# UmbertoDellaMonica/fp-mash

Hardware: AMD Instinct MI355X
Metric: bases/s sketched + Mpairs/s dist, k=21 s=1000, 1/2/4/8 MI355X; %HBM roofline (higher is better)
Workload: dtype u64; 1 GPU; n_seqs_per_gpu=10000, seq_len=2000, k=21, s=1000, pairs_per_gpu=100000000, listed_pairs_per_gpu=1000006, full=False

## Files before the change

fp-mash_amd/csrc/dist.hip:

```cpp
#include "fpm_device.hpp"
#include "fpm_kernels.hpp"

#pragma clang fp contract(off)

#include <cstdlib>

#include <float.h>

#include <algorithm>

namespace fpm {

constexpr int kTile = 16;
constexpr int kWalkBlk = 4;

template <typename H>
__device__ __forceinline__ void walk_pair(const H *__restrict__ A, uint32_t la,
                                          const H *__restrict__ B, uint32_t lb, uint32_t S,
                                          uint32_t &numer, uint32_t &denom)
{
    uint32_t i = 0, j = 0, common = 0, d = 0;
    H a = la ? A[0] : H(0), b = lb ? B[0] : H(0);
    while (d < S && i < la && j < lb) {
        const bool lt = a < b, gt = b < a;
        if (!gt) { i++; if (i < la) a = A[i]; }
        if (!lt) { j++; if (j < lb) b = B[j]; }
        common += (!lt && !gt) ? 1u : 0u;
        d++;
    }
    if (d < S) {
        uint64_t dd = (uint64_t)d + (la - i) + (lb - j);
        d = dd > S ? S : (uint32_t)dd;
    }
    numer = common;
    denom = d;
}

template <typename H, typename C>
__global__ __launch_bounds__(256) void compare_grid_kernel(
    const H *__restrict__ ref, const uint32_t *__restrict__ ref_len, uint64_t ref_stride,
    uint32_t n_ref, const H *__restrict__ qry, const uint32_t *__restrict__ qry_len,
    uint64_t qry_stride, uint32_t n_qry, uint32_t S, C *__restrict__ numer,
    C *__restrict__ denom)
{
    const uint32_t r = blockIdx.x * kTile + (threadIdx.x & (kTile - 1));
    const uint32_t q = blockIdx.y * kTile + (threadIdx.x / kTile);
    if (r >= n_ref || q >= n_qry) return;
    uint32_t c, d;
    walk_pair(ref + (uint64_t)r * ref_stride, ref_len[r], qry + (uint64_t)q * qry_stride,
              qry_len[q], S, c, d);
    const uint64_t o = (uint64_t)q * n_ref + r;
    numer[o] = (C)c;
    denom[o] = (C)d;
}

__device__ __forceinline__ uint32_t lane_sel(uint32_t x, uint32_t y, uint64_t m)
{
    uint32_t r;
    asm("v_cndmask_b32_e64 %0, %1, %2, %3" : "=v"(r) : "v"(x), "v"(y), "s"(m));
    return r;
}
__device__ __forceinline__ uint64_t lane_sel(uint64_t x, uint64_t y, uint64_t m)
{
    return ((uint64_t)lane_sel((uint32_t)(x >> 32), (uint32_t)(y >> 32), m) << 32) |
           lane_sel((uint32_t)x, (uint32_t)y, m);
}

template <typename H, int BLK, typename C>
__global__ __launch_bounds__(256) void compare_grid_lds_kernel(
    const H *__restrict__ ref, const uint32_t *__restrict__ ref_len, uint64_t ref_stride,
    uint32_t n_ref, const H *__restrict__ qry, const uint32_t *__restrict__ qry_len,
    uint64_t qry_stride, uint32_t n_qry, uint32_t S, uint32_t W, C *__restrict__ numer,
    C *__restrict__ denom)
{
    extern __shared__ __attribute__((aligned(16))) unsigned char smem[];
    H *lds = reinterpret_cast<H *>(smem);
    __shared__ uint32_t cnt[2 * kTile];
    const uint32_t Wp = (W + BLK + 3) & ~3u;
    const uint32_t r0 = blockIdx.x * kTile, q0 = blockIdx.y * kTile;
    if (threadIdx.x < 2 * kTile) {
        const uint32_t l = threadIdx.x, isq = l >= (uint32_t)kTile, row = (isq ? q0 : r0) + (l & (kTile - 1));
        uint32_t c = 0;
        if (row < (isq ? n_qry : n_ref)) c = isq ? qry_len[row] : ref_len[row];
        cnt[l] = c < W ? c : W;
    }
    __syncthreads();
    const uint32_t wave = threadIdx.x >> 6, lane = threadIdx.x & 63;
    constexpr uint32_t kV = 16 / sizeof(H);
    constexpr int kL = 2 * kTile / 4;
    const bool vec = ((ref_stride * sizeof(H)) & 15) == 0 && ((qry_stride * sizeof(H)) & 15) == 0 &&
                     (((uintptr_t)ref | (uintptr_t)qry) & 15) == 0;
    if (vec) {
// ... 107 lines not shown
        if (++x < na) ra = RA[x];
        if (++y < nb) rb = RB[y];
    }
    numer = common;
    const uint64_t dd = (uint64_t)la + lb - common;
    denom = dd > S ? S : (uint32_t)dd;
}

template <typename H, typename C>
__global__ __launch_bounds__(256) void walk_cand_kernel(
    const uint64_t *__restrict__ cand, const unsigned long long *__restrict__ n_cand,
    const H *__restrict__ ref, const uint32_t *__restrict__ ref_len, uint64_t ref_stride,
    uint32_t n_ref, const H *__restrict__ qry, const uint32_t *__restrict__ qry_len,
    uint64_t qry_stride, uint32_t S, RecRows rr, RecRows rq, C *__restrict__ numer,
    C *__restrict__ denom)
{
    const uint64_t idx = (uint64_t)blockIdx.x * blockDim.x + threadIdx.x;
    if (idx >= *n_cand) return;
    const uint64_t o = cand[idx];
    const uint32_t q = (uint32_t)(o / n_ref), r = (uint32_t)(o % n_ref);
    uint32_t c, d;
    const H *A = ref + (uint64_t)r * ref_stride, *B = qry + (uint64_t)q * qry_stride;
    if (A == B && ref_len[r] == qry_len[q]) {
        const uint32_t l = ref_len[r];
        c = l < S ? l : S;
        const uint64_t dd = 2ull * l - c;
        d = dd > S ? S : (uint32_t)dd;
    } else if (rr.val)
        walk_pair_rec(ref + (uint64_t)r * ref_stride, ref_len[r], qry + (uint64_t)q * qry_stride,
                      qry_len[q], S, (const H *)rr.val + (uint64_t)r * rr.stride,
                      rr.pos + (uint64_t)r * rr.stride, rr.len[r],
                      (const H *)rq.val + (uint64_t)q * rq.stride, rq.pos + (uint64_t)q * rq.stride,
                      rq.len[q], c, d);
    else
        walk_pair(ref + (uint64_t)r * ref_stride, ref_len[r], qry + (uint64_t)q * qry_stride,
                  qry_len[q], S, c, d);
    numer[o] = (C)c;
    denom[o] = (C)d;
}

constexpr int kRankWaves = 4;
constexpr int kRankProbeMax = 8;
constexpr uint32_t kRankLogB = 12;

template <int NP, bool HI = false>
__device__ __forceinline__ uint64_t rank_chunk(const uint64_t *Bs, const uint32_t *K32,
                                               const uint16_t *Bkt, uint32_t shift,
                                               uint32_t kshift, uint32_t top, uint32_t lb,
                                               uint32_t maxn, uint32_t kb, uint64_t a, uint32_t &j)
{
    bool over;
    uint32_t lo;
    if constexpr (HI) {
        over = false;
        lo = Bkt[min((uint32_t)(a >> 32) >> (shift - 32), kb)];
    } else {
        const uint64_t t = a >> shift;
        over = t > (uint64_t)top;
        lo = Bkt[over ? top + 1 : (uint32_t)t];
    }
    if constexpr (NP > 0) {
        const uint32_t ka = HI ? (uint32_t)(a >> 32) : (uint32_t)(a >> kshift);
        uint32_t p = lo;
#pragma unroll
        for (int q = 0; q < NP; q++) p += K32[lo + q] < ka ? 1u : 0u;
        const uint64_t v = Bs[p];
        j = p + (v < a ? 1u : 0u);
        if constexpr (HI) return __builtin_amdgcn_ballot_w64(v == a);
        return __builtin_amdgcn_ballot_w64(v == a) & ~__builtin_amdgcn_ballot_w64(over);
    } else {
        uint32_t jj = lo;
        uint64_t eqm = 0;
        for (uint32_t q = 0; q < maxn; q++) {
            const uint32_t p = min(lo + q, lb);
            const uint64_t v = Bs[p];
            jj += ((v < a) & (p < lb)) ? 1u : 0u;
            eqm |= __builtin_amdgcn_ballot_w64((v == a) & (p < lb));
        }
        j = jj;
        return eqm;
    }
}

template <int CAP, typename C>
__global__ __launch_bounds__(64 * kRankWaves) void rank_rows_kernel(
    const uint64_t *__restrict__ cand, const uint64_t *__restrict__ row_seg, uint32_t n_qry,
    uint32_t q_lo, const uint64_t *__restrict__ ref, const uint32_t *__restrict__ ref_len,
    uint64_t ref_stride, uint32_t n_ref, const uint64_t *__restrict__ qry,
    const uint32_t *__restrict__ qry_len, uint64_t qry_stride, uint32_t S, uint32_t sym,
    C *__restrict__ numer, C *__restrict__ denom, uint32_t *__restrict__ cnum,
    uint32_t *__restrict__ cden)
{
    constexpr uint32_t kLogBuckets = (CAP <= 1024) ? kRankLogB : kRankLogB + 1;
    constexpr uint32_t kBuckets = 1u << kLogBuckets;
    __shared__ struct {
        uint32_t k[CAP + kRankProbeMax];
        uint64_t v[CAP + kRankProbeMax];
    } sKB;
    uint32_t *const K32 = sKB.k;
    uint64_t *const Bs = sKB.v;
    __shared__ uint16_t Bkt[kBuckets + 1];
    __shared__ uint32_t s_maxn, s_keydup, s_unsorted;
    const uint32_t qr = xcd_row(blockIdx.x, n_qry);
    if (qr >= n_qry) return;
    const uint32_t q = q_lo + qr;
    const uint64_t seg = row_seg[q];
    const uint32_t n = (uint32_t)(seg & 0xFFFFFF);
    if (n == 0) return;
    const uint64_t base = seg >> 24;
    const uint32_t lane = threadIdx.x & 63, wave = __builtin_amdgcn_readfirstlane(threadIdx.x >> 6);
    const uint32_t lb = qry_len[q];
    const uint64_t *B = qry + (uint64_t)q * qry_stride;
    if (threadIdx.x == 0) { s_maxn = 0; s_keydup = 0; s_unsorted = 0; }
    {
        constexpr int kStage = (CAP + 64 * kRankWaves - 1) / (64 * kRankWaves);
        uint64_t v[kStage];
#pragma unroll
        for (int u = 0; u < kStage; u++) {
            const uint32_t t = threadIdx.x + u * 64 * kRankWaves;
            v[u] = t < lb ? B[t] : 0;
        }
#pragma unroll
        for (int u = 0; u < kStage; u++) {
            const uint32_t t = threadIdx.x + u * 64 * kRankWaves;
            if (t < lb) Bs[t] = v[u];
        }
    }
    if (threadIdx.x < kRankProbeMax) {
        Bs[lb + threadIdx.x] = ~0ULL;
        K32[lb + threadIdx.x] = 0xFFFFFFFFu;
    }
    __syncthreads();
    const uint64_t bmax = lb ? Bs[lb - 1] : 0;
    const uint32_t bits = bmax ? 64 - __clzll(bmax) : 0;
    const uint32_t shift = bits > kLogBuckets ? bits - kLogBuckets : 0;
    const uint32_t kshift = shift >= 32 ? 32 : bits > 32 ? bits - 32 : 0;
    const uint32_t top = (uint32_t)(bmax >> shift);
    uint32_t dup = 0, uns = 0;
    for (uint32_t j = threadIdx.x; j <= lb; j += blockDim.x) {
        const uint64_t v = j < lb ? Bs[j] : 0, vp = j > 0 ? Bs[j - 1] : 0;
        if (j < lb) {
            const uint32_t k = (uint32_t)(v >> kshift);
            K32[j] = k;
            dup |= (j > 0 && (uint32_t)(vp >> kshift) == k) | (k == 0xFFFFFFFFu);
            uns |= j > 0 && !(vp < v);
        }
        const uint32_t bj = j < lb ? (uint32_t)(v >> shift) : top + 1;
        const uint32_t bp = j > 0 ? (uint32_t)(vp >> shift) + 1 : 0;
        for (uint32_t b = bp; b <= bj; b++) Bkt[b] = (uint16_t)j;
    }
    for (uint32_t b = top + 2 + threadIdx.x; b <= kBuckets; b += blockDim.x) Bkt[b] = (uint16_t)lb;
    if (dup) s_keydup = 1;
    if (uns) s_unsorted = 1;
    __syncthreads();
    if (s_unsorted) return;
    uint32_t mx = 0;
    for (uint32_t j = threadIdx.x; j < lb; j += blockDim.x)
        mx = max(mx, j + 1 - (uint32_t)Bkt[(uint32_t)(Bs[j] >> shift)]);
#pragma unroll
    for (int d = 32; d > 0; d >>= 1) mx = max(mx, (uint32_t)__shfl_xor(mx, d, 64));
    if (lane == 0 && mx) atomicMax(&s_maxn, mx);
    __syncthreads();
    const uint32_t maxn = s_maxn;
    const uint32_t np = s_keydup ? 0u
                      : maxn <= 2 ? 2u : maxn <= 3 ? 3u : maxn <= 4 ? 4u
                      : maxn <= (uint32_t)kRankProbeMax ? (uint32_t)kRankProbeMax : 0u;

    const uint32_t ld = ref_stride < (uint64_t)CAP ? (uint32_t)ref_stride : (uint32_t)CAP;
    const uint64_t pair_row = (uint64_t)q * n_ref;
    constexpr int kGroup = 1;
    constexpr uint32_t kChunk = 128;
    struct Row { __amdgpu_buffer_rsrc_t rsrc; uint32_t la; uint64_t o; };
    auto open_row = [&](uint64_t o) -> Row {
        const uint32_t rr = __builtin_amdgcn_readfirstlane((uint32_t)(o - pair_row));
        const uintptr_t Ar = (uintptr_t)(ref + (uint64_t)rr * ref_stride);
        const uint32_t plo = __builtin_amdgcn_readfirstlane((uint32_t)Ar);
        const uint32_t phi = __builtin_amdgcn_readfirstlane((uint32_t)(Ar >> 32));
        Row R;
        R.rsrc = __builtin_amdgcn_make_buffer_rsrc((void *)(((uintptr_t)phi << 32) | plo), 0,
                                                   (int)__builtin_amdgcn_readfirstlane(ld * 8u),
                                                   0x00020000);
        R.la = ref_len[rr];
        R.o = o;
        return R;
    };
    struct Pair { uint64_t e0, e1; };
    auto load_group = [&](const Row &R, uint32_t gi, Pair (&dst)[kGroup]) {
#pragma unroll
        for (int u = 0; u < kGroup; u++) {
            const uint32_t t = gi * kGroup + u;
            const auto v0 = __builtin_amdgcn_raw_buffer_load_b64(R.rsrc, (t * kChunk + lane) * 8u, 0, 0);
            const auto v1 = __builtin_amdgcn_raw_buffer_load_b64(R.rsrc, (t * kChunk + 64 + lane) * 8u,
                                                                 0, 0);
            dst[u].e0 = ((uint64_t)v0[1] << 32) | v0[0];
            dst[u].e1 = ((uint64_t)v1[1] << 32) | v1[0];
        }
    };
    auto cand_at = [&](uint32_t cc) -> uint64_t {
        return cand[base + __builtin_amdgcn_readfirstlane(cc)];
    };
    auto rank_group = [&](auto probe, uint32_t g0, bool last, uint64_t vm0, uint64_t vm1,
                          const Pair (&cur)[kGroup], uint32_t &shared_below,
                          uint32_t &cnt) -> uint32_t {
        uint32_t j0, j1;
        const uint64_t m0 = probe(cur[0].e0, j0);
        const uint64_t m1 = probe(cur[0].e1, j1);
        const uint32_t i0 = g0 * kChunk;
        const uint64_t a0 = m0 & vm0, a1 = m1 & vm1;
        const uint32_t p0 = (uint32_t)__popcll(a0), p1 = (uint32_t)__popcll(a1);
        uint32_t u_last = 0;
        if (!last) {
            const uint32_t jl = (uint32_t)__builtin_amdgcn_readlane((int)j1, 63);
            u_last = i0 + (kChunk - 1) + jl -
                     (shared_below + p0 + (uint32_t)__popcll(a1 & 0x7FFFFFFFFFFFFFFFULL));
        }
        if (!last && u_last < S) {
            cnt += p0 + p1;
        } else {
            const uint32_t b0 = __builtin_amdgcn_mbcnt_hi(
                (uint32_t)(a0 >> 32), __builtin_amdgcn_mbcnt_lo((uint32_t)a0, 0u));
            const uint32_t b1 = __builtin_amdgcn_mbcnt_hi(
                (uint32_t)(a1 >> 32), __builtin_amdgcn_mbcnt_lo((uint32_t)a1, 0u));
            const uint32_t k0 = shared_below + b0;
            const uint32_t k1 = shared_below + p0 + b1;
            const uint32_t u0 = i0 + lane + j0 - k0, u1 = i0 + 64 + lane + j1 - k1;
            cnt += __popcll(a0 & __builtin_amdgcn_ballot_w64(u0 < S)) +
                   __popcll(a1 & __builtin_amdgcn_ballot_w64(u1 < S));
        }
        shared_below += p0 + p1;
        return u_last;
    };
    auto run = [&](auto probe, bool fast) {
        Pair cur[kGroup], nxt[kGroup], pf[kGroup];
        Row Rc{};
        if (wave < n) { Rc = open_row(cand_at(wave)); load_group(Rc, 0, pf); }
        for (uint32_t c = wave; c < n; c += kRankWaves) {
            const Row R = Rc;
#pragma unroll
            for (int u = 0; u < kGroup; u++) cur[u] = pf[u];
            if (c + kRankWaves < n) { Rc = open_row(cand_at(c + kRankWaves)); load_group(Rc, 0, pf); }
            const uint32_t la = R.la;
            const uint64_t o = R.o;
            const bool need_all = la < S && lb < S;
            const uint32_t nch = (la + kChunk - 1) / kChunk;
            const uint32_t ngr = (nch + kGroup - 1) / kGroup;
            static_assert(kGroup == 1, "the last-chunk masks assume one chunk per group");
            const int rl = (int)la - (int)(nch - 1) * (int)kChunk;
            const int r0 = min(rl, 64), r1 = rl - 64;
            const uint64_t vl0 = r0 >= 64 ? ~0ULL : r0 > 0 ? (1ULL << r0) - 1 : 0ULL;
            const uint64_t vl1 = r1 >= 64 ? ~0ULL : r1 > 0 ? (1ULL << r1) - 1 : 0ULL;
            uint32_t shared_below = 0, cnt = 0;
            const uint32_t s_exit = need_all ? 0xFFFFFFFFu : S;
            bool exited = false;
            uint32_t gi = 0;
            for (; gi + 1 < ngr; gi++) {
                load_group(R, gi + 1, nxt);
                const uint32_t u_last = rank_group(probe, gi * kGroup, false, ~0ULL, ~0ULL, cur,
                                                   shared_below, cnt);
                if (u_last >= s_exit) { exited = true; break; }
#pragma unroll
                for (int u = 0; u < kGroup; u++) cur[u] = nxt[u];
            }
            if (!exited && ngr) {
                const uint64_t x0 = fast ? __builtin_amdgcn_ballot_w64(cur[0].e0 == ~0ULL) : 0;
                const uint64_t x1 = fast ? __builtin_amdgcn_ballot_w64(cur[0].e1 == ~0ULL) : 0;
                rank_group(probe, gi * kGroup, true, vl0 & ~x0, vl1 & ~x1, cur, shared_below, cnt);
            }
            if (lane == 0) {
                const uint64_t un = (uint64_t)la + lb - shared_below;
                const uint32_t dn = need_all ? (un < S ? (uint32_t)un : S) : S;
                if (cnum) {
                    cnum[base + c] = cnt;
                    cden[base + c] = dn;
                    continue;
                }
                numer[o] = (C)cnt;
                denom[o] = (C)dn;
                const uint32_t r = (uint32_t)(o - pair_row);
                if (sym && r != q) {
                    const uint64_t o2 = (uint64_t)r * n_ref + q;
                    numer[o2] = (C)cnt;
                    denom[o2] = (C)dn;
                }
            }
        }
    };
    const uint16_t *bk_ = Bkt;
    const uint64_t *bs_ = Bs;
    const uint32_t *k_ = K32;
#define FPM_RANK_NP(NP_, HI_) \
    run([&](uint64_t a, uint32_t &j) { \
        return rank_chunk<NP_, HI_>(bs_, k_, bk_, shift, kshift, top, lb, maxn, kBuckets, a, j); }, NP_ > 0)
    const bool hi = shift >= 32;
    switch (np) {
    case 2: if (hi) FPM_RANK_NP(2, true); else FPM_RANK_NP(2, false); break;
    case 3: if (hi) FPM_RANK_NP(3, true); else FPM_RANK_NP(3, false); break;
    case 4: if (hi) FPM_RANK_NP(4, true); else FPM_RANK_NP(4, false); break;
    case kRankProbeMax: FPM_RANK_NP(kRankProbeMax, false); break;
    default: FPM_RANK_NP(0, false); break;
    }
#undef FPM_RANK_NP
}

template <typename C>
static hipError_t merge_rows_c(const uint64_t *d_cand, const uint64_t *row_seg, uint32_t n_qry,
                               const uint64_t *d_ref, const uint32_t *d_ref_len,
                               uint64_t ref_stride, uint32_t n_ref, const uint64_t *d_qry,
                               const uint32_t *d_qry_len, uint64_t qry_stride, uint32_t S,
                               bool sym, C *d_numer, C *d_denom, uint32_t *d_cnum,
                               uint32_t *d_cden, hipStream_t st, uint32_t q_lo,
                               uint32_t *rank_cap)
{
    const dim3 g(xcd_grid(n_qry)), b(64 * kRankWaves);
    const uint64_t cap = std::max(ref_stride, qry_stride);
    if (rank_cap) *rank_cap = cap <= 1024 ? 1024u : 2048u;
    if (cap <= 1024)
        hipLaunchKernelGGL((rank_rows_kernel<1024, C>), g, b, 0, st, d_cand, row_seg, n_qry, q_lo,
                           d_ref, d_ref_len, ref_stride, n_ref, d_qry, d_qry_len, qry_stride, S,
                           (uint32_t)sym, d_numer, d_denom, d_cnum, d_cden);
    else if (cap <= 2048)
        hipLaunchKernelGGL((rank_rows_kernel<2048, C>), g, b, 0, st, d_cand, row_seg, n_qry, q_lo,
                           d_ref, d_ref_len, ref_stride, n_ref, d_qry, d_qry_len, qry_stride, S,
                           (uint32_t)sym, d_numer, d_denom, d_cnum, d_cden);
    else
        return hipErrorInvalidValue;
    return hipGetLastError();
}

hipError_t launch_merge_rows(const uint64_t *d_cand, const uint64_t *row_seg, uint32_t n_qry,
                             const uint64_t *d_ref, const uint32_t *d_ref_len, uint64_t ref_stride,
                             uint32_t n_ref, const uint64_t *d_qry, const uint32_t *d_qry_len,
                             uint64_t qry_stride, uint32_t S, bool sym, Counts cnt,
                             uint32_t *d_cnum, uint32_t *d_cden, hipStream_t st, uint32_t q_lo,
                             uint32_t *rank_cap)
{
    if (!n_qry) return hipSuccess;
    if (cnt.c16)
        return merge_rows_c(d_cand, row_seg, n_qry, d_ref, d_ref_len, ref_stride, n_ref, d_qry,
                            d_qry_len, qry_stride, S, sym, (uint16_t *)cnt.numer,
                            (uint16_t *)cnt.denom, d_cnum, d_cden, st, q_lo, rank_cap);
    return merge_rows_c(d_cand, row_seg, n_qry, d_ref, d_ref_len, ref_stride, n_ref, d_qry,
                        d_qry_len, qry_stride, S, sym, (uint32_t *)cnt.numer,
                        (uint32_t *)cnt.denom, d_cnum, d_cden, st, q_lo, rank_cap);
}


__device__ double lngs_large(double x)
{
    double x2 = 1.0 / (x * x);
    double s = (1.0 / 12.0) - x2 * ((1.0 / 360.0) - x2 * ((1.0 / 1260.0) - x2 * ((1.0 / 1680.0)
               - x2 * ((1.0 / 1188.0) - x2 * ((691.0 / 360360.0) - x2 * (1.0 / 156.0))))));
    return s / x;
}

__device__ double lngammastar(double x)
{
    if (x >= 10.0) return lngs_large(x);
    double n = ceil(10.0 - x), y = x + n, prod = 1.0;
    for (double t = x; t < y - 0.5; t += 1.0) prod *= t;
    double lg = lngs_large(y) + (y - 0.5) * log(y) - y - log(prod);
    return lg - ((x - 0.5) * log(x) - x);
}

__device__ double lnbeta(double a, double b)
{
    double s = a + b;
    double t = -(a - 0.5) * log1p(b / a) - (b - 0.5) * log1p(a / b) - 0.5 * log(s);
    return lngammastar(a) + lngammastar(b) - lngammastar(s) + 0.91893853320467274178 + t;
}

__device__ double beta_cf(double a, double b, double x, double epsabs)
{
    const double cutoff = 2.0 * DBL_MIN;
    unsigned it = 0;
    double num = 1.0, den = 1.0 - (a + b) * x / (a + 1.0);
    if (fabs(den) < cutoff) den = __builtin_nan("");
    den = 1.0 / den;
    double cf = den;
    while (it < 512) {
        const int k = (int)it + 1;
        double coeff = k * (b - k) * x / (((a - 1.0) + 2 * k) * (a + 2 * k));
        den = 1.0 + coeff * den;
        num = 1.0 + coeff / num;
        if (fabs(den) < cutoff) den = __builtin_nan("");
        if (fabs(num) < cutoff) num = __builtin_nan("");
        den = 1.0 / den;
        double delta = den * num;
        cf *= delta;
        coeff = -(a + k) * (a + b + k) * x / ((a + 2 * k) * (a + 2 * k + 1.0));
        den = 1.0 + coeff * den;
        num = 1.0 + coeff / num;
        if (fabs(den) < cutoff) den = __builtin_nan("");
        if (fabs(num) < cutoff) num = __builtin_nan("");
        den = 1.0 / den;
        delta = den * num;
        cf *= delta;
        if (fabs(delta - 1.0) < 2.0 * DBL_EPSILON) break;
        if (cf * fabs(delta - 1.0) < epsabs) break;
        ++it;
    }
    if (it >= 512) return __builtin_nan("");
    return cf;
}

__device__ double lngamma_pos(double x)
{
    return lngammastar(x) + (x - 0.5) * log(x) - x + 0.91893853320467274178;
}

__device__ __forceinline__ double gamma_inc_PQ(double a, double x, bool upper)
{
    if (x <= 0.0) return upper ? 1.0 : 0.0;
    if (x < a + 1.0) {
        double sum = 1.0, term = 1.0;
        for (int n = 1; n < 100000; n++) {
            term *= x / (a + n);
            sum += term;
            if (term < sum * DBL_EPSILON) break;
        }
        const double P = exp(a * log(x) - x - lngamma_pos(a + 1.0)) * sum;
        return upper ? 1.0 - P : P;
    }
    const double tiny = 1e-300;
    double b = x + 1.0 - a, c = 1.0 / tiny, d = 1.0 / b, h = d;
    for (int i = 1; i < 100000; i++) {
        const double an = -(double)i * ((double)i - a);
// ... 1154 lines not shown
```

fp-mash_amd/csrc/dist_index.hip:

```cpp
#include "fpm_device.hpp"
#include "fpm_kernels.hpp"

#include <algorithm>
#include <atomic>

namespace fpm {

constexpr uint32_t kParts = 1u << kIdxL1;
#ifndef PROBE_KU
#define PROBE_KU 8
#endif

__device__ __forceinline__ uint64_t load_key(const void *lists, uint32_t hash_bytes, uint64_t idx)
{
    return hash_bytes == 8 ? reinterpret_cast<const uint64_t *>(lists)[idx]
                           : (uint64_t) reinterpret_cast<const uint32_t *>(lists)[idx];
}

__device__ __forceinline__ uint64_t norm_key(uint64_t h, uint32_t hash_bytes)
{
    return hash_bytes == 8 ? h : (h << 32);
}

__device__ __forceinline__ uint64_t idx_mult(const IdxGeom &g)
// ... 501 lines not shown
#pragma unroll
        for (int d = 1; d < 64; d <<= 1) { uint32_t y = __shfl_up(x, d, 64); if (lane >= d) x += y; }
        if (lane == 63) wsum[wave] = x;
        __syncthreads();
        uint32_t wpre = 0;
        for (int w = 0; w < wave; w++) wpre += wsum[w];
        if (i < nb) sums[i] = carry + wpre + x - v;
        __syncthreads();
        if (threadIdx.x == 255) carry += wpre + x;
        __syncthreads();
    }
    if (threadIdx.x == 0 && total) *total = carry;
}

__global__ __launch_bounds__(256) void scan_add_kernel(uint32_t *__restrict__ out, uint64_t n,
                                                      const uint32_t *__restrict__ sums,
                                                      uint32_t *__restrict__ out2)
{
    const uint64_t base = (uint64_t)blockIdx.x * kScanBlock + threadIdx.x * 4;
    const uint32_t add = sums[blockIdx.x];
#pragma unroll
    for (int k = 0; k < 4; k++)
        if (base + k < n) {
            uint32_t v = out[base + k] + add;
            out[base + k] = v;
            if (out2) out2[base + k] = v;
        }
}

constexpr uint32_t kPC = 4;
__global__ __launch_bounds__(256) void probe_count_kernel(
    const void *__restrict__ qry, const uint32_t *__restrict__ qry_len, uint64_t stride,
    uint32_t n_qry, uint32_t hash_bytes, IdxGeom g, const uint32_t *__restrict__ dir,
    unsigned long long *__restrict__ events, uint32_t *__restrict__ unsorted)
{
    __shared__ unsigned long long wsum[4];
    const uint64_t n = (uint64_t)n_qry * stride;
    const uint64_t e0 = ((uint64_t)blockIdx.x * blockDim.x + threadIdx.x) * kPC;
    uint64_t ev = 0;
    uint32_t uns = 0;
    if (e0 < n) {
        uint32_t q = (uint32_t)(e0 / stride), j = (uint32_t)(e0 - (uint64_t)q * stride);
        uint64_t key[kPC + 1];
        uint32_t jj[kPC], lq[kPC];
        bool ok[kPC + 1];
#pragma unroll
        for (uint32_t u = 0; u <= kPC; u++) {
            const uint32_t l = q < n_qry ? qry_len[q] : 0u;
            ok[u] = j < l;
            key[u] = ok[u] ? load_key(qry, hash_bytes, (uint64_t)q * stride + j) : 0;
            if (u < kPC) { jj[u] = j; lq[u] = l; }
            if (++j == stride) { j = 0; q++; }
        }
        uint32_t d0[kPC], d1[kPC];
#pragma unroll
        for (uint32_t u = 0; u < kPC; u++) {
            const uint64_t b = bucket_of(norm_key(key[u], hash_bytes), g, idx_mult(g));
            d0[u] = ok[u] ? dir[b] : 0u;
            d1[u] = ok[u] ? dir[b + 1] : 0u;
        }
#pragma unroll
        for (uint32_t u = 0; u < kPC; u++) {
            ev += d1[u] - d0[u];
            if (ok[u] && jj[u] + 1 < lq[u] && !(key[u] < key[u + 1])) uns = 1;
        }
    }
    for (int d = 32; d > 0; d >>= 1) ev += __shfl_down(ev, d, 64);
    if ((threadIdx.x & 63) == 0) wsum[threadIdx.x >> 6] = ev;
    if (__any(uns) && (threadIdx.x & 63) == 0) atomicOr(unsorted, 1u);
    __syncthreads();
    if (threadIdx.x == 0) {
        unsigned long long t = wsum[0] + wsum[1] + wsum[2] + wsum[3];
        if (t) atomicAdd(&events[1 + (blockIdx.x & 63)], t);
    }
}

__global__ void sum64_kernel(unsigned long long *events)
{
    unsigned long long v = events[1 + threadIdx.x];
    for (int d = 32; d > 0; d >>= 1) v += __shfl_down(v, d, 64);
    if (threadIdx.x == 0) events[0] = v;
}

template <typename C, bool HALF>
__global__ __launch_bounds__(256) __attribute__((amdgpu_waves_per_eu(8)))
void probe_rows_kernel(
    const void *__restrict__ qry, const uint32_t *__restrict__ qry_len, uint64_t stride,
    uint32_t n_qry, uint32_t q_lo, uint32_t n_ref, uint32_t hash_bytes, IdxGeom g,
    const uint32_t *__restrict__ dir, const uint32_t *__restrict__ entries,
    uint32_t chunk_refs, const uint32_t *__restrict__ ref_len, uint32_t S, uint32_t sym,
    uint32_t defaults, uint32_t vec_defaults, uint32_t self_set, C *__restrict__ numer,
    C *__restrict__ denom, uint64_t *__restrict__ cand,
    unsigned long long *__restrict__ n_cand, uint64_t *__restrict__ row_seg,
    const uint32_t *__restrict__ qry_it_len, uint32_t *__restrict__ q_unsorted,
    unsigned long long *__restrict__ events, uint64_t cap, uint32_t *__restrict__ cand_over)
{
    extern __shared__ __attribute__((aligned(16))) uint32_t rowbits[];
    __shared__ uint32_t wsum[4];
    __shared__ unsigned long long row_base;
    constexpr uint32_t kWin = 1024;
    __shared__ uint64_t w_tab[4][64];
    __shared__ uint8_t w_own[4][kWin];
    const uint32_t qr = xcd_row(blockIdx.x, n_qry);
    if (qr >= n_qry) return;
    const uint32_t q = q_lo + qr;
    const uint64_t mult = idx_mult(g);
    const uint32_t r0 = blockIdx.y * chunk_refs;
    const uint32_t r1 = min(n_ref, r0 + chunk_refs);
    auto word_mask = [&](uint32_t w) -> uint32_t {
        if (!sym) return ~0u;
        const uint32_t rb = r0 + 32 * w;
        const uint32_t odd = ((q ^ rb) & 1u) ? 0x55555555u : 0xAAAAAAAAu;
        const uint32_t gt = q < rb ? ~0u : q - rb >= 31 ? 0u : ~((2u << (q - rb)) - 1u);
        return (odd & gt) | (~odd & ~gt);
    };
    const uint32_t nwords = (r1 - r0 + 31) / 32;
    const uint32_t both0 = nwords * 32;
    for (uint32_t w = threadIdx.x; w < nwords * (HALF ? 2 : 1); w += 256) rowbits[w] = 0;
    __syncthreads();
    const uint32_t lq = qry_len[q];
    const uint32_t lit = HALF ? (lq >= S ? (S + 1) / 2 : lq) : qry_it_len ? qry_it_len[q] : lq;
    if (self_set && threadIdx.x == 0 && lq > 0 && q >= r0 && q < r1)
        atomicOr(&rowbits[(q - r0) >> 5], 1u << ((q - r0) & 31));
    const uint64_t rowoff = (uint64_t)q * stride;
    const uint32_t lane = threadIdx.x & 63, wave = threadIdx.x >> 6;
    const uint32_t rmask = (uint32_t)((1ULL << g.rbits) - 1);
    constexpr int kB = 4;
    uint64_t ev_w = 0;
    uint32_t uns = 0;
    for (uint32_t jb = wave * 64; jb < lit; jb += 256 * kB) {
        uint32_t st_b[kB], cnt_b[kB], tgt_b[kB];
#pragma unroll
        for (int bi = 0; bi < kB; bi++) {
            const uint32_t j = jb + 256 * bi + lane;
            const uint64_t raw = j < lit ? load_key(qry, hash_bytes, rowoff + j) : 0;
            if (!HALF && q_unsorted) {
                uint64_t nx = __shfl_down(raw, 1, 64);
                if (lane == 63 && j + 1 < lit) nx = load_key(qry, hash_bytes, rowoff + j + 1);
                if (j + 1 < lit && !(raw < nx)) uns = 1;
            }
            const uint64_t K = j < lit ? norm_key(raw, hash_bytes) : 0;
            const uint64_t b = bucket_of(K, g, mult);
            const uint32_t d0 = j < lit ? dir[b] : 0u, d1 = j < lit ? dir[b + 1] : 0u;
            st_b[bi] = d0;
            cnt_b[bi] = self_set && d1 - d0 == 1 ? 0u : d1 - d0;
            tgt_b[bi] = key_fp(K, g, mult);
        }
#pragma unroll
      for (int bi = 0; bi < kB; bi++) {
        if (jb + 256 * bi >= lit) break;
        const uint32_t st = st_b[bi], cnt = cnt_b[bi], tgt = tgt_b[bi];
        uint32_t inc = cnt;
#pragma unroll
        for (int d = 1; d < 64; d <<= 1) {
            const uint32_t y = __shfl_up(inc, d, 64);
            if ((int)lane >= d) inc += y;
        }
        const uint32_t total = __builtin_amdgcn_readlane(inc, 63);
        ev_w += total;
        const uint32_t pre = inc - cnt;
        w_tab[wave][lane] = ((uint64_t)tgt << 32) | (uint32_t)(st - pre);
        for (uint32_t wb = 0; wb < total; wb += kWin) {
            const uint32_t a0 = max(pre, wb), a1 = min(pre + cnt, wb + kWin);
            for (uint32_t e = a0; e < a1; e++) w_own[wave][e - wb] = (uint8_t)lane;
            __builtin_amdgcn_wave_barrier();
            const uint32_t wn = min(kWin, total - wb);
            constexpr int kU = PROBE_KU;
            for (uint32_t e0 = lane; e0 < wn; e0 += 64 * kU) {
                uint64_t tab[kU];
#pragma unroll
                for (int u = 0; u < kU; u++) {
                    const uint32_t e = e0 + 64 * u;
                    tab[u] = w_tab[wave][w_own[wave][e < wn ? e : 0]];
                }
                uint32_t en[kU];
#pragma unroll
                for (int u = 0; u < kU; u++) {
                    const uint32_t e = e0 + 64 * u;
                    en[u] = e < wn ? entries[(uint32_t)tab[u] + wb + e] : 0u;
                }
                uint32_t wi[kU], need = 0;
#pragma unroll
                for (int u = 0; u < kU; u++) {
                    const uint32_t e = e0 + 64 * u;
                    const uint32_t r = en[u] & rmask;
                    const bool hit = e < wn &&
                                     ((en[u] & ~kEntryFlag) >> g.rbits) == (uint32_t)(tab[u] >> 32) &&
                                     r >= r0 && r < r1;
                    wi[u] = hit ? r - r0 : 0u;
                    if (HALF) wi[u] += hit && (en[u] & kEntryFlag) ? both0 : 0u;
                    const uint32_t word = rowbits[wi[u] >> 5];
                    need |= (hit && !(word & (1u << (wi[u] & 31)))) ? (1u << u) : 0u;
                }
                if (__any(need != 0)) {
#pragma unroll
                    for (int u = 0; u < kU; u++)
                        if (need >> u & 1u) {
                            atomicOr(&rowbits[wi[u] >> 5], 1u << (wi[u] & 31));
                            if (HALF && wi[u] >= both0)
                                atomicOr(&rowbits[(wi[u] - both0) >> 5], 1u << (wi[u] & 31));
                        }
                }
            }
            __builtin_amdgcn_wave_barrier();
        }
        __builtin_amdgcn_wave_barrier();
      }
    }
    if (!HALF && q_unsorted && __any(uns) && lane == 0) atomicOr(q_unsorted, 1u);
    if (!HALF && events && blockIdx.y == 0 && lane == 0 && ev_w)
        atomicAdd(&events[1 + (blockIdx.x & 63)], ev_w);
    __syncthreads();
    auto taken = [&](uint32_t w) -> uint32_t {
        const uint32_t m = word_mask(w);
        if (!HALF) return rowbits[w] & m;
        const uint32_t seen = rowbits[w], both = rowbits[nwords + w];
        return (seen & m) | (seen & ~both & ~m);
    };
    uint32_t mycnt = 0;
    for (uint32_t w = threadIdx.x; w < nwords; w += 256) mycnt += __popc(taken(w));
    uint32_t x = mycnt;
#pragma unroll
    for (int d = 1; d < 64; d <<= 1) { uint32_t y = __shfl_up(x, d, 64); if (lane >= d) x += y; }
    if (lane == 63) wsum[wave] = x;
    __syncthreads();
    uint32_t wpre = 0, tot = 0;
    for (uint32_t w = 0; w < 4; w++) { if (w < wave) wpre += wsum[w]; tot += wsum[w]; }
    if (threadIdx.x == 0) {
        row_base = tot ? atomicAdd(n_cand, (unsigned long long)tot) : 0ULL;
        const bool over = row_base + tot > cap;
        if (over) atomicOr(cand_over, 1u);
        if (gridDim.y == 1) row_seg[q] = (row_base << 24) | (over ? 0u : (tot & 0xFFFFFF));
        if (over) row_base = ~0ULL;
    }
    __syncthreads();
    const bool dropped = row_base == ~0ULL;
    uint64_t pos = row_base + wpre + x - mycnt;
    const uint64_t pair_row = (uint64_t)q * n_ref;
    for (uint32_t w = threadIdx.x; !dropped && w < nwords; w += 256) {
        uint32_t b = taken(w);
        const uint64_t bit0 = pair_row + r0 + (uint64_t)w * 32;
        while (b) {
            int t = __builtin_ctz(b);
            b &= b - 1;
            cand[pos++] = bit0 + t;
        }
    }
    if (defaults) {
        if (vec_defaults) {
            for (uint32_t r = r0 + threadIdx.x * 4; r < r1; r += 1024) {
                const uint64_t o = pair_row + r;
                const uint4 rl = *(const uint4 *)(ref_len + r);
                const uint32_t d0 = rl.x + lq, d1 = rl.y + lq, d2 = rl.z + lq, d3 = rl.w + lq;
                typedef unsigned int u32x2 __attribute__((ext_vector_type(2)));
                typedef unsigned int u32x4 __attribute__((ext_vector_type(4)));
                if constexpr (sizeof(C) == 2) {
                    __builtin_nontemporal_store(u32x2{0u, 0u}, (u32x2 *)(numer + o));
                    __builtin_nontemporal_store(u32x2{min(d0, S) | (min(d1, S) << 16),
                                                      min(d2, S) | (min(d3, S) << 16)},
                                                (u32x2 *)(denom + o));
                } else {
                    __builtin_nontemporal_store(u32x4{0u, 0u, 0u, 0u}, (u32x4 *)(numer + o));
                    __builtin_nontemporal_store(u32x4{min(d0, S), min(d1, S), min(d2, S), min(d3, S)},
                                                (u32x4 *)(denom + o));
                }
            }
        } else {
            for (uint32_t r = r0 + threadIdx.x; r < r1; r += 256) {
                const uint64_t o = pair_row + r;
                const uint64_t d = (uint64_t)ref_len[r] + lq;
                numer[o] = 0;
                denom[o] = (C)(d < S ? (uint32_t)d : S);
            }
        }
    }
}

constexpr int kRecWaves = 4;
template <typename H>
__global__ __launch_bounds__(64 * kRecWaves) void record_rows_kernel(
    const H *__restrict__ in, const uint32_t *__restrict__ in_len, uint64_t in_stride, uint32_t n,
    uint32_t S, H *__restrict__ out, uint32_t *__restrict__ pos_out, uint32_t *__restrict__ out_len,
    uint64_t out_stride, uint32_t *__restrict__ unsorted)
{
    const uint32_t lane = threadIdx.x & 63;
    const uint32_t row = blockIdx.x * kRecWaves + (threadIdx.x >> 6);
    if (row >= n) return;
    if (unsorted) {
        const uint32_t len = in_len[row];
        const H *r = in + (uint64_t)row * in_stride;
        bool uns = false;
        for (uint32_t c0 = 0; c0 < len; c0 += 64) {
            const uint32_t i = c0 + lane;
            const H v = i < len ? r[i] : H(0);
            H nx = (H)__shfl_down((unsigned long long)v, 1, 64);
            if (lane == 63 && i + 1 < len) nx = r[i + 1];
            uns |= i + 1 < len && !(v < nx);
        }
        if (__any(uns) && lane == 0) atomicOr(unsorted, 1u);
    }
    const uint32_t m = min(min(in_len[row], S), (uint32_t)out_stride);
    const H *src = in + (uint64_t)row * in_stride;
    H *dst = out + (uint64_t)row * out_stride;
    uint32_t *pdst = pos_out ? pos_out + (uint64_t)row * out_stride : nullptr;
    H run = 0;
    uint32_t cnt = 0;
    for (uint32_t c0 = 0; c0 < m; c0 += 64) {
        const uint32_t i = c0 + lane;
        const H v = i < m ? src[i] : H(0);
        H pm = v;
#pragma unroll
        for (int d = 1; d < 64; d <<= 1) {
            const H y = (H)__shfl_up((unsigned long long)pm, d, 64);
            if ((int)lane >= d) pm = pm > y ? pm : y;
        }
        H before = (H)__shfl_up((unsigned long long)pm, 1, 64);
        before = lane == 0 ? run : (before > run ? before : run);
        const bool rec = i < m && (i == 0 || v > before);
        const uint64_t bm = __ballot(rec);
        const uint32_t at = cnt + __builtin_amdgcn_mbcnt_hi((uint32_t)(bm >> 32),
                                                            __builtin_amdgcn_mbcnt_lo((uint32_t)bm, 0u));
        if (rec) dst[at] = v;
        if (rec && pdst) pdst[at] = i;
        cnt += (uint32_t)__popcll(bm);
        const H top = (H)__shfl((unsigned long long)pm, 63, 64);
        run = top > run ? top : run;
    }
    if (lane == 0) out_len[row] = cnt;
// ... 14 lines not shown
        hipLaunchKernelGGL(record_rows_kernel<uint32_t>, g, b, 0, st, (const uint32_t *)in, in_len,
                           in_stride, n, S, (uint32_t *)out, pos_out, out_len, out_stride,
                           unsorted);
    return hipGetLastError();
}

__global__ __launch_bounds__(kPubWords) void publish_kernel(const unsigned long long *__restrict__ src,
                                                          uint32_t n, unsigned long long *dst,
                                                          unsigned long long seq)
{
    unsigned long long ev = (threadIdx.x >= 1 && threadIdx.x <= 64 && n > 64) ? src[threadIdx.x] : 0;
    for (int d = 32; d > 0; d >>= 1) ev += __shfl_xor(ev, d, 64);
    __shared__ unsigned long long wsum[kPubWords / 64];
    if ((threadIdx.x & 63) == 0) wsum[threadIdx.x >> 6] = ev;
    __syncthreads();
    if (threadIdx.x == 0 && n > 64) {
        unsigned long long t = 0;
        for (uint32_t w = 0; w < kPubWords / 64; w++) t += wsum[w];
        dst[0] = t;
    } else if (threadIdx.x < n) {
        dst[threadIdx.x] = src[threadIdx.x];
    }
    __threadfence_system();
    __syncthreads();
    if (threadIdx.x == 0) __hip_atomic_store(dst + kPubWords - 1, seq, __ATOMIC_RELEASE,
                                             __HIP_MEMORY_SCOPE_SYSTEM);
}

hipError_t launch_publish(const unsigned long long *d_src, uint32_t n, unsigned long long *h_dst,
                          unsigned long long seq, hipStream_t st)
{
    if (n >= kPubWords) return hipErrorInvalidValue;
    hipLaunchKernelGGL(publish_kernel, dim3(1), dim3(kPubWords), 0, st, d_src, n, h_dst, seq);
    return hipGetLastError();
}

constexpr uint32_t kScanFoldBlocks = 4096;
__global__ __launch_bounds__(256) void scan_add_fold_kernel(uint32_t *__restrict__ out, uint64_t n,
                                                           const uint32_t *__restrict__ sums,
                                                           uint32_t nb, uint32_t *__restrict__ out2,
                                                           uint32_t *__restrict__ total)
{
    __shared__ uint32_t wsum[4];
    const uint32_t b = blockIdx.x;
    uint32_t part = 0;
    for (uint32_t i = threadIdx.x; i < b; i += 256) part += sums[i];
#pragma unroll
    for (int d = 32; d > 0; d >>= 1) part += __shfl_xor(part, d, 64);
    if ((threadIdx.x & 63) == 0) wsum[threadIdx.x >> 6] = part;
    __syncthreads();
    const uint32_t add = wsum[0] + wsum[1] + wsum[2] + wsum[3];
    if (total && b == nb - 1 && threadIdx.x == 0) *total = add + sums[b];
    const uint64_t base = (uint64_t)b * kScanBlock + threadIdx.x * 4;
#pragma unroll
    for (int k = 0; k < 4; k++)
        if (base + k < n) {
            const uint32_t v = out[base + k] + add;
            out[base + k] = v;
            if (out2) out2[base + k] = v;
        }
}

uint64_t scan_scratch_words(uint64_t n) { return (n + kScanBlock - 1) / kScanBlock + 1; }

hipError_t launch_exscan(const uint32_t *in, uint32_t *out, uint32_t *out2, uint64_t n,
                         uint32_t *scratch, uint32_t *total, hipStream_t st)
{
    if (!n) return hipSuccess;
    uint32_t nb = (uint32_t)((n + kScanBlock - 1) / kScanBlock);
    hipLaunchKernelGGL(scan_local_kernel, dim3(nb), dim3(256), 0, st, in, out, n, scratch);
    if (nb <= kScanFoldBlocks) {
        hipLaunchKernelGGL(scan_add_fold_kernel, dim3(nb), dim3(256), 0, st, out, n,
                           (const uint32_t *)scratch, nb, out2, total);
        return hipGetLastError();
    }
    hipLaunchKernelGGL(scan_sums_kernel, dim3(1), dim3(256), 0, st, scratch, nb, total);
    hipLaunchKernelGGL(scan_add_kernel, dim3(nb), dim3(256), 0, st, out, n, scratch, out2);
    return hipGetLastError();
}

static hipError_t dyn_lds_attr(int slot, const void *fn, int bytes)
{
    constexpr int kMaxDev = 64;
    static std::atomic<int> done[5][kMaxDev];
    int dev = 0;
    if (hipError_t e = hipGetDevice(&dev)) return e;
    if (dev < 0 || dev >= kMaxDev) return hipFuncSetAttribute(fn, hipFuncAttributeMaxDynamicSharedMemorySize, bytes);
    if (done[slot][dev].load(std::memory_order_acquire)) return hipSuccess;
    hipError_t e = hipFuncSetAttribute(fn, hipFuncAttributeMaxDynamicSharedMemorySize, bytes);
    if (e == hipSuccess) done[slot][dev].store(1, std::memory_order_release);
    return e;
}

uint64_t idx_tent_words(const IdxGeom &g, uint64_t E)
{
    return g.cap ? (uint64_t)kParts * g.cap : E;
}

hipError_t launch_idx_build(const void *d_ref, const uint32_t *d_ref_len, uint64_t stride,
                            uint32_t n_ref, uint32_t hash_bytes, IdxGeom g, uint32_t *tile_hist,
                            uint32_t *tile_off, uint32_t *scan_s, uint64_t *tent,
                            uint32_t *dir, uint32_t *entries, uint32_t *unsorted,
                            unsigned long long *self_events, unsigned long long *zero,
                            uint32_t nzero, unsigned long long *acc, uint32_t *part_fill,
                            uint32_t *overflow, hipStream_t st, unsigned long long *zero_x,
                            unsigned long long *n_entries)
{
    if (g.vcut && !g.cut) return hipErrorInvalidValue;
    const uint32_t ntiles = g.ntiles;
    const uint64_t magic = stride > 1 ? ~0ULL / stride + 1 : 0;
    const uint32_t kg = std::max<uint32_t>(1, std::min<uint32_t>(
        (n_ref + kKmaxThreads * kKmaxU - 1) / (kKmaxThreads * kKmaxU), 64));
    const bool one_pass = g.cap != 0 && part_fill && overflow;
    hipLaunchKernelGGL(idx_kmax_kernel, dim3(kg), dim3(kKmaxThreads), 0, st, d_ref, d_ref_len,
                       stride, n_ref, hash_bytes, (unsigned long long *)g.kmax, zero, nzero, acc,
                       one_pass ? part_fill : nullptr, one_pass ? kParts : 0u, zero_x,
                       g.vcut ? g.cut : 0u, n_entries);
    uint32_t lsplit = 0;
    const double part_mean = (double)n_ref * (double)stride / (double)kParts;
    while (lsplit < g.l2 && lsplit < 4 &&
           (((uint64_t)4 << (g.l2 - lsplit)) > 32768 || part_mean / (double)(1u << lsplit) > 24576.0))
        lsplit++;
    const uint64_t cnt_bytes0 = (uint64_t)4 << (g.l2 - lsplit);
    constexpr uint32_t kLdsBytes = 159 * 1024;
    const uint32_t lds_cap = part_mean / (double)(1u << lsplit) <= 12288.0
                                 ? (uint32_t)(kBucketThreads * kBucketPer)
                                 : (uint32_t)((kLdsBytes - cnt_bytes0) / 4);
    const dim3 bgrid(kParts << lsplit);
    if (hipError_t e = dyn_lds_attr(1, (const void *)idx_bucket_kernel, kLdsBytes))
        return e;
    if (one_pass) {
        if (hipError_t e = dyn_lds_attr(2, (const void *)idx_part_scatter1_kernel, kIdxTile * 8))
            return e;
        hipLaunchKernelGGL(idx_part_scatter1_kernel, dim3(ntiles), dim3(kIdxThreads),
                           (size_t)g.tile * 8, st, d_ref, d_ref_len, (uint32_t)stride, magic,
                           n_ref, hash_bytes, g, part_fill, tent, unsorted, overflow);
        hipLaunchKernelGGL(idx_bucket_kernel, bgrid, dim3(kBucketThreads),
                           (size_t)(cnt_bytes0 + (uint64_t)lds_cap * 4), st, (const uint64_t *)tent,
                           ntiles, (const uint32_t *)nullptr, g, lds_cap, dir, entries, self_events,
                           (const uint32_t *)part_fill, lsplit, n_entries);
        return hipGetLastError();
    }
    hipLaunchKernelGGL(idx_part_hist_kernel, dim3(ntiles), dim3(kIdxThreads), 0, st, d_ref,
                       d_ref_len, (uint32_t)stride, magic, n_ref, hash_bytes, ntiles, tile_hist,
                       unsorted, g);
    const uint64_t nh = (uint64_t)kParts * ntiles;
    if (hipError_t e = launch_exscan(tile_hist, tile_off, nullptr, nh, scan_s, tile_off + nh, st))
        return e;
    if (hipError_t e = dyn_lds_attr(0, (const void *)idx_part_scatter_kernel, kIdxTile * 8))
        return e;
    hipLaunchKernelGGL(idx_part_scatter_kernel, dim3(ntiles), dim3(kIdxThreads),
                       (size_t)g.tile * 8, st, d_ref, d_ref_len, (uint32_t)stride, magic, n_ref,
                       hash_bytes, ntiles, (const uint32_t *)tile_hist, (const uint32_t *)tile_off,
                       g, tent);
    hipLaunchKernelGGL(idx_bucket_kernel, bgrid, dim3(kBucketThreads),
                       (size_t)(cnt_bytes0 + (uint64_t)lds_cap * 4), st, (const uint64_t *)tent,
                       ntiles, (const uint32_t *)tile_off, g, lds_cap, dir, entries, self_events,
                       (const uint32_t *)nullptr, lsplit, n_entries);
    return hipGetLastError();
}

hipError_t launch_probe_count(const void *d_qry, const uint32_t *d_qry_len, uint64_t stride,
                              uint32_t n_qry, uint32_t hash_bytes, IdxGeom g, const uint32_t *dir,
                              unsigned long long *events, uint32_t *unsorted, hipStream_t st)
{
    uint64_t n = (uint64_t)n_qry * stride;
    const uint64_t threads = (n + kPC - 1) / kPC;
    if (n) hipLaunchKernelGGL(probe_count_kernel, dim3((uint32_t)((threads + 255) / 256)), dim3(256),
                              0, st, d_qry, d_qry_len, stride, n_qry, hash_bytes, g, dir, events,
                              unsorted);
    return hipGetLastError();
}

hipError_t launch_probe_rows(const void *d_qry, const uint32_t *d_qry_len, uint64_t stride,
                             uint32_t n_qry, uint32_t n_ref, uint32_t hash_bytes, IdxGeom g,
                             const uint32_t *dir, const uint32_t *entries,
                             const uint32_t *d_ref_len, uint32_t S, bool sym, bool defaults,
                             bool self_set, Counts cnt, uint64_t *cand,
                             unsigned long long *n_cand, uint64_t *row_seg,
                             const uint32_t *d_qry_it_len, uint32_t *q_unsorted,
                             unsigned long long *events, uint64_t cap, uint32_t *cand_over,
                             hipStream_t st, uint32_t q_lo, bool half)
{
    if (!n_qry || !n_ref) return hipSuccess;
    if (half && (!sym || !self_set || g.cut != S || d_qry_it_len || q_unsorted || events))
        return hipErrorInvalidValue;
    const uint32_t chunk = 1u << 19;
    const uint32_t nchunks = (n_ref + chunk - 1) / chunk;
    const uint32_t cref = nchunks == 1 ? n_ref : chunk;
    const size_t lds = ((cref + 31) / 32) * 4 * (half ? 2 : 1);
    if (lds > 64 * 1024) {
        const void *fn = cnt.c16 ? (const void *)probe_rows_kernel<uint16_t, true>
                                 : (const void *)probe_rows_kernel<uint32_t, true>;
        if (hipError_t e = dyn_lds_attr(cnt.c16 ? 3 : 4, fn, 128 * 1024)) return e;
    }
    const auto al = [](const void *p) { return ((uintptr_t)p & 15) == 0; };
    const uint32_t vec_defaults = n_ref % 4 == 0 && cref % 4 == 0 && al(d_ref_len) &&
                                  al(cnt.numer) && al(cnt.denom);
#define FPM_PROBE(C, H)                                                                         \
    hipLaunchKernelGGL((probe_rows_kernel<C, H>), dim3(xcd_grid(n_qry), nchunks), dim3(256), lds, \
                       st, d_qry, d_qry_len, stride, n_qry, q_lo, n_ref, hash_bytes, g, dir,     \
                       entries, cref,                                                            \
                       d_ref_len, S, (uint32_t)sym, (uint32_t)defaults, vec_defaults,           \
                       (uint32_t)self_set, (C *)cnt.numer, (C *)cnt.denom, cand, n_cand, row_seg, \
                       d_qry_it_len, q_unsorted, events, cap, cand_over)
    if (cnt.c16 && half) FPM_PROBE(uint16_t, true);
    else if (cnt.c16) FPM_PROBE(uint16_t, false);
    else if (half) FPM_PROBE(uint32_t, true);
    else FPM_PROBE(uint32_t, false);
#undef FPM_PROBE
    return hipGetLastError();
}

}
```

fp-mash_amd/csrc/fpm_ctx.cpp:

```cpp
#include "fpm_internal.hpp"

#include <atomic>
#include <cstdlib>

static thread_local std::string g_err;

int fail(int code, const std::string &msg)
{
    g_err = msg;
    return code;
}

hipError_t pool_alloc(fpm_ctx *ctx, void **p, size_t bytes)
{
    {
        std::lock_guard<std::mutex> g(ctx->pool_mu);
        size_t best = SIZE_MAX, bi = 0;
        for (size_t i = 0; i < ctx->pool.size(); i++) {
            const size_t b = ctx->pool[i].second;
            if (b >= bytes && b <= 4 * bytes + 4096 && b < best) { best = b; bi = i; }
            if (best == bytes) break;
        }
        if (best != SIZE_MAX) {
            *p = ctx->pool[bi].first;
// ... 162 lines not shown
                std::atomic_thread_fence(std::memory_order_seq_cst);
                if (*flag != seq) return fail(FPM_EHIP, "counter publish did not land");
            }
        }
        __builtin_ia32_pause();
    }
    std::atomic_thread_fence(std::memory_order_acquire);
    return FPM_OK;
}

int read_counters(fpm_ctx *ctx, const unsigned long long *d_src, uint32_t n,
                         hipStream_t st)
{
    unsigned long long seq;
    if (int rc = publish_counters(ctx, d_src, n, st, &seq)) return rc;
    return wait_counters(ctx, seq, st);
}

hipError_t grow_slot(fpm_ctx::Slot &s, size_t bytes, void **out)
{
    if (s.bytes < bytes) {
        if (s.p) { hipError_t e = hipFree(s.p); if (e != hipSuccess) return e; }
        s.p = nullptr;
        s.bytes = 0;
        size_t b = bytes + bytes / 8 + 256;
        hipError_t e = hipMalloc(&s.p, b);
        if (e != hipSuccess) return e;
        s.bytes = b;
    }
    *out = s.p;
    return hipSuccess;
}

hipError_t scratch(fpm_ctx *ctx, ScratchSlot id, size_t bytes, void **out)
{
    auto &s = ctx->scratch[id];
    const bool grows = s.bytes < bytes;
    hipError_t e = grow_slot(s, bytes, out);
    if (e == hipSuccess && grows && s.bytes <= 4096) e = memset_sync(ctx, s.p, 0, s.bytes);
    return e;
}

int set_device(fpm_ctx *ctx)
{
    if (!ctx) return fail(FPM_EINVAL, "null context");
    HIP_TRY(hipSetDevice(ctx->device));
    return FPM_OK;
}

extern "C" {

int fpm_abi_version(void) { return FPM_ABI_VERSION; }

const char *fpm_last_error(void) { return g_err.c_str(); }

int fpm_device_count(int *count)
{
    if (!count) return fail(FPM_EINVAL, "null count");
    int n = 0;
    hipError_t e = hipGetDeviceCount(&n);
    if (e != hipSuccess) n = 0;
    *count = n;
    return FPM_OK;
}

int fpm_ctx_create(int device, fpm_ctx **out)
{
    if (!out) return fail(FPM_EINVAL, "null out");
    *out = nullptr;
    int n = 0;
    if (hipGetDeviceCount(&n) != hipSuccess || n == 0)
        return fail(FPM_ENODEV, "no HIP device visible (fpmash has no CPU fallback)");
    if (device < 0 || device >= n) return fail(FPM_EINVAL, "device index out of range");
    hipDeviceProp_t prop;
    HIP_TRY(hipGetDeviceProperties(&prop, device));
    if (std::string(prop.gcnArchName).rfind("gfx950", 0) != 0)
        return fail(FPM_ENODEV, std::string("device is ") + prop.gcnArchName +
                                    ", fpmash kernels are built for gfx950 only");
    fpm_ctx *ctx = new fpm_ctx();
    ctx->device = device;
    if (const char *v = getenv("FPM_FILL_COUNTS")) ctx->fill_counts = atoi(v) != 0 ? 1 : 0;
    if (const char *v = getenv("FPM_PROBE_HALF")) ctx->probe_half = atoi(v) != 0;
    if (const char *v = getenv("FPM_INDEX_CUT")) ctx->index_cut = atoi(v) != 0;
    hipError_t e = hipSetDevice(device);
    if (e == hipSuccess) e = hipStreamCreateWithFlags(&ctx->stream, hipStreamNonBlocking);
    if (e != hipSuccess) {
        delete ctx;
        return fail(FPM_EHIP, std::string("context init: ") + hipGetErrorString(e));
    }
    *out = ctx;
    return FPM_OK;
}

void fpm_ctx_destroy(fpm_ctx *ctx)
{
    if (!ctx) return;
    (void)hipSetDevice(ctx->device);
    fpm_ctx_reset_timing(ctx);
    for (auto &s : ctx->scratch)
        if (s.p) (void)hipFree(s.p);
    if (ctx->host_counters) (void)hipHostFree(ctx->host_counters);
    if (ctx->stream) (void)hipStreamDestroy(ctx->stream);
    if (ctx->aux) (void)hipStreamDestroy(ctx->aux);
    if (ctx->ev_in) (void)hipEventDestroy(ctx->ev_in);
    if (ctx->ev_fill) (void)hipEventDestroy(ctx->ev_fill);
    if (ctx->ev_prefill) (void)hipEventDestroy(ctx->ev_prefill);
    for (int i = 0; i < fpm_ctx::kRing; i++) {
        if (ctx->ring[i]) (void)hipHostFree(ctx->ring[i]);
        if (ctx->ring_ev[i]) (void)hipEventDestroy(ctx->ring_ev[i]);
    }
    for (auto &b : ctx->pool) (void)hipFree(b.first);
    delete ctx;
}

int fpm_ctx_warm(fpm_ctx *ctx)
{
    if (int rc = set_device(ctx)) return rc;
    HIP_TRY(ensure_ring(ctx));
    constexpr size_t kWarm = 1u << 20;
    void *d = nullptr;
    HIP_TRY(hipMalloc(&d, kWarm));
    hipError_t e = hipMemcpyAsync(d, ctx->ring[0], kWarm, hipMemcpyHostToDevice, ctx->stream);
    if (e == hipSuccess) e = hipMemcpyAsync(ctx->ring[1], d, kWarm, hipMemcpyDeviceToHost, ctx->stream);
    if (e == hipSuccess) e = hipStreamSynchronize(ctx->stream);
    const hipError_t f = hipFree(d);
    HIP_TRY(e);
    HIP_TRY(f);
    return FPM_OK;
}

void *fpm_ctx_stream(fpm_ctx *ctx) { return ctx ? (void *)ctx->stream : nullptr; }

int fpm_stream_create(fpm_ctx *ctx, void **stream)
{
    if (!stream) return fail(FPM_EINVAL, "null stream");
    if (int rc = set_device(ctx)) return rc;
    hipStream_t s = nullptr;
    HIP_TRY(hipStreamCreateWithFlags(&s, hipStreamNonBlocking));
    *stream = s;
    return FPM_OK;
}

int fpm_stream_destroy(fpm_ctx *ctx, void *stream)
{
    if (int rc = set_device(ctx)) return rc;
    if (stream) HIP_TRY(hipStreamDestroy((hipStream_t)stream));
    return FPM_OK;
}

int fpm_event_create(fpm_ctx *ctx, void **event)
{
    if (!event) return fail(FPM_EINVAL, "null event");
    if (int rc = set_device(ctx)) return rc;
    hipEvent_t e = nullptr;
    HIP_TRY(hipEventCreateWithFlags(&e, hipEventDisableTiming));
    *event = e;
    return FPM_OK;
}

int fpm_event_destroy(fpm_ctx *ctx, void *event)
{
    if (int rc = set_device(ctx)) return rc;
    if (event) HIP_TRY(hipEventDestroy((hipEvent_t)event));
    return FPM_OK;
}

// ... 64 lines not shown
    if (int rc = set_device(ctx)) return rc;
    if (bytes) HIP_TRY(hipMemsetAsync(dptr, value, bytes, ctx->stream));
    HIP_TRY(hipStreamSynchronize(ctx->stream));
    return FPM_OK;
}

int fpm_host_alloc(fpm_ctx *ctx, void **p, size_t bytes)
{
    if (!p) return fail(FPM_EINVAL, "host_alloc: null output");
    *p = nullptr;
    if (int rc = set_device(ctx)) return rc;
    if (hipHostMalloc(p, bytes ? bytes : 16) != hipSuccess)
        return fail(FPM_ENOMEM, "host_alloc: pinned allocation failed");
    return FPM_OK;
}

int fpm_host_free(fpm_ctx *ctx, void *p)
{
    if (int rc = set_device(ctx)) return rc;
    if (p) HIP_TRY(hipHostFree(p));
    return FPM_OK;
}

int fpm_ctx_set_dist_mode(fpm_ctx *ctx, int mode)
{
    if (!ctx || mode < FPM_DIST_AUTO || mode > FPM_DIST_SPARSE) return fail(FPM_EINVAL, "bad dist mode");
    ctx->dist_mode = mode;
    return FPM_OK;
}

int fpm_ctx_last_dist_stats(fpm_ctx *ctx, int *sparse, uint64_t *events, uint64_t *candidates)
{
    if (!ctx) return fail(FPM_EINVAL, "null context");
    if (sparse) *sparse = ctx->last_sparse;
    if (events) *events = ctx->last_events;
    if (ctx->last_cand == (uint64_t)-1) {
        if (int rc = set_device(ctx)) return rc;
        HIP_TRY(hipStreamSynchronize(ctx->last_cand_stream));
        unsigned long long v = 0;
        HIP_TRY(hipMemcpy(&v, ctx->last_cand_dev, 8, hipMemcpyDeviceToHost));
        ctx->last_cand = v;
    }
    if (candidates) *candidates = ctx->last_cand;
    return FPM_OK;
}

int fpm_ctx_last_dist_kernel(fpm_ctx *ctx, int *kernel)
{
    if (!ctx || !kernel) return fail(FPM_EINVAL, "null argument");
    *kernel = ctx->last_kernel;
    return FPM_OK;
}

int fpm_ctx_set_probe_half(fpm_ctx *ctx, int on)
{
    if (!ctx) return fail(FPM_EINVAL, "null context");
    ctx->probe_half = on != 0;
    return FPM_OK;
}

int fpm_ctx_last_dist_probe(fpm_ctx *ctx, int *form)
{
    if (!ctx || !form) return fail(FPM_EINVAL, "null argument");
    *form = ctx->last_probe;
    return FPM_OK;
}

int fpm_ctx_set_index_cut(fpm_ctx *ctx, int on)
{
    if (!ctx) return fail(FPM_EINVAL, "null context");
    ctx->index_cut = on != 0;
    return FPM_OK;
}

int fpm_ctx_last_index_cut(fpm_ctx *ctx, int *cut, uint64_t *indexed, uint64_t *entries)
{
    if (!ctx) return fail(FPM_EINVAL, "null context");
    if (cut) *cut = ctx->last_index_cut ? 1 : 0;
    if (indexed) *indexed = ctx->last_indexed;
    if (entries) *entries = ctx->last_entries;
    return FPM_OK;
}

int fpm_ctx_index_rebuilds(fpm_ctx *ctx, uint64_t *count)
{
    if (!ctx || !count) return fail(FPM_EINVAL, "null argument");
    *count = ctx->idx_rebuilds;
    return FPM_OK;
}

int fpm_ctx_spec_stats(fpm_ctx *ctx, uint64_t *hits, uint64_t *misses)
{
    if (!ctx || !hits || !misses) return fail(FPM_EINVAL, "null argument");
    *hits = ctx->spec_hits;
    *misses = ctx->spec_misses;
    return FPM_OK;
}

int fpm_ctx_set_timing(fpm_ctx *ctx, int enable)
{
    if (!ctx) return fail(FPM_EINVAL, "null context");
    ctx->timing = enable != 0;
    return FPM_OK;
}

int fpm_ctx_reset_timing(fpm_ctx *ctx)
{
    if (!ctx) return fail(FPM_EINVAL, "null context");
    for (auto &v : ctx->ev) {
        for (auto &pr : v) {
            (void)hipEventDestroy(pr.first);
            (void)hipEventDestroy(pr.second);
        }
        v.clear();
    }
    return FPM_OK;
}

int fpm_ctx_kernel_time(fpm_ctx *ctx, int kernel, double *total_ms, uint64_t *launches)
{
    if (!ctx || kernel < 0 || kernel >= FPM_K_COUNT) return fail(FPM_EINVAL, "bad kernel id");
    if (int rc = set_device(ctx)) return rc;
    double t = 0;
    for (auto &pr : ctx->ev[kernel]) {
        HIP_TRY(hipEventSynchronize(pr.second));
        float ms = 0;
        HIP_TRY(hipEventElapsedTime(&ms, pr.first, pr.second));
        t += ms;
    }
    if (total_ms) *total_ms = t;
    if (launches) *launches = ctx->ev[kernel].size();
    return FPM_OK;
}

}
```

fp-mash_amd/csrc/fpm_dist_api.cpp:

```cpp
#include "fpm_internal.hpp"

#include <cmath>
#include <cstdlib>
#include <functional>
#include <memory>

struct RowSet {
    const void *rows;
    const uint32_t *len;
    const uint64_t *length;
    uint64_t stride;
    uint32_t n;
};

struct DistParams {
    uint32_t kmer_size;
    double kmer_space, max_dist, max_pvalue;
};

struct DistOut {
    Counts cnt;
    double *dist = nullptr, *pval = nullptr;
    uint8_t *pass = nullptr;
    CellList list{};
// ... 107 lines not shown
    const uint32_t *entries() const { return (const uint32_t *)slot[kEntries].p; }
};

static int refset_build_index(fpm_refset *rs, hipStream_t st)
{
    fpm_ctx *ctx = rs->ctx;
    const RowSet &R = rs->ref;
    const uint64_t E = (uint64_t)R.n * R.stride;
    IdxGeom geom = make_geom(R.n, E, rs->sketch_size);
    rs->sparse_ok = E > 0 && geom.rbits <= 24 && E < (1ULL << 31);
    if (!rs->sparse_ok) return FPM_OK;
    void *ctr;
    HIP_TRY(scratch(ctx, kSlotCounters, kCtrWords * 8, &ctr));
    if (!rs->kmax) HIP_TRY(hipMalloc((void **)&rs->kmax, 8));
    auto build = [&](const RowSet &rows, IdxGeom &g, bool raw) -> int {
        void *dir, *entries;
        HIP_TRY(grow_slot(rs->slot[fpm_refset::kDir], ((1ULL << g.nbits) + 1) * 4, &dir));
        HIP_TRY(grow_slot(rs->slot[fpm_refset::kEntries], (uint64_t)R.n * rows.stride * 4, &entries));
        return build_index(ctx, rows, rs->hash_bytes, g, (uint32_t *)dir, (uint32_t *)entries,
                           (unsigned long long *)ctr, true, st, [] { return FPM_OK; }, raw);
    };
    geom.kmax = rs->kmax;
    if (int rc = build(R, geom, true)) return rc;
    rs->ref_unsorted = host_unsorted(ctx);
    rs->self_events = host_events(ctx);
    rs->n_indexed = host_indexed(ctx);
    rs->mr =std::min<uint64_t>(R.stride, rs->sketch_size);
    rs->recorded = rs->ref_unsorted;
    if (rs->recorded) {
        void *dref, *dref_len, *dref_pos;
        HIP_TRY(grow_slot(rs->slot[fpm_refset::kRecRows], (size_t)R.n * rs->mr * rs->hash_bytes, &dref));
        HIP_TRY(grow_slot(rs->slot[fpm_refset::kRecLen], (size_t)R.n * 4, &dref_len));
        HIP_TRY(grow_slot(rs->slot[fpm_refset::kRecPos], (size_t)R.n * rs->mr * 4, &dref_pos));
        {
            TimedLaunch tl(ctx, FPM_K_INDEX, st);
            HIP_TRY(launch_record_rows(R.rows, R.len, R.stride, R.n, rs->hash_bytes,
                                       rs->sketch_size, dref, (uint32_t *)dref_pos,
                                       (uint32_t *)dref_len, rs->mr, st));
            tl.done();
        }
        geom = make_geom(R.n, (uint64_t)R.n * rs->mr, 0);
        geom.kmax = rs->kmax;
        if (int rc = build(RowSet{dref, (const uint32_t *)dref_len, nullptr, rs->mr, R.n}, geom,
                           false))
            return rc;
        rs->n_indexed = host_indexed(ctx);
    }
    rs->geom = geom;
    return FPM_OK;
}


struct Compare {
    fpm_ctx *ctx;
    hipStream_t st;
    RowSet R, Q;
    uint32_t hash_bytes, S;
    Counts cnt;
    const DistFinal *fin;
    fpm_refset *rs;
    uint64_t n_pairs;
    bool self_set, compact, want_mir;
    bool prefilled, fill_cnt, need_fill;
    unsigned long long *list_cnt;
    bool list_zeroed;
    bool prefill_done;
    bool fill_pending = false;
    bool probe_defaults() const { return !fill_cnt && !prefilled; }
};

struct SparsePlan {
    unsigned long long *ctr = nullptr;
    IdxGeom geom{};
    const uint32_t *dir = nullptr, *entries = nullptr;
    const void *p_rows = nullptr;
    const uint32_t *p_len = nullptr;
    uint64_t p_stride = 0;
    uint64_t ev = 0;
    bool all_sorted = true;
    RecRows rec_r{}, rec_q{};
    bool skip_count = false;
    bool spec_probe = false;
    bool spec_half = false;
    unsigned long long *n_cand() const { return ctr + kCtrCand; }
    uint32_t *unsorted() const { return (uint32_t *)(ctr + kCtrUnsorted); }
    uint32_t *cand_over() const { return (uint32_t *)(ctr + kCtrCandOver); }
};

static bool probe_half(const Compare &c, const SparsePlan &p, bool sym)
{
    return sym && c.ctx->probe_half && p.geom.cut == c.S && !p.p_len && !p.skip_count;
}

static bool index_cut_ok(const Compare &c)
{
    return c.ctx->index_cut && c.ctx->probe_half && !c.rs && c.self_set && c.hash_bytes == 8 &&
           c.S > 0 && c.R.n <= (1u << 19) && std::max(c.R.stride, c.Q.stride) <= 2048;
}

static uint64_t whole_index_events(uint64_t ev, uint64_t entries, uint64_t indexed)
{
    if (!indexed || indexed >= entries) return ev;
    const unsigned __int128 x = (unsigned __int128)ev * entries + (indexed - 1);
    const unsigned __int128 q = x / indexed;
    return q > (unsigned __int128)UINT64_MAX ? UINT64_MAX : (uint64_t)q;
}

static void note_index(fpm_ctx *ctx, const IdxGeom &g)
{
    ctx->last_index_cut = g.vcut != 0;
    ctx->last_indexed = host_indexed(ctx);
    ctx->last_entries = host_entries(ctx);
}

static int zero_list(Compare &c)
{
    if (!c.list_zeroed) HIP_TRY(hipMemsetAsync(c.list_cnt, 0, 8, c.st));
    c.list_zeroed = true;
    return FPM_OK;
}

static int settle_prefill(Compare &c)
{
    if (c.prefill_done) return FPM_OK;
    c.prefill_done = true;
    HIP_TRY(hipStreamWaitEvent(c.st, c.ctx->ev_prefill, 0));
    HIP_TRY(launch_dist_counts_fixup(c.R.len, c.R.n, c.Q.len, c.Q.n, c.S, (uint16_t *)c.cnt.denom,
                                     c.st));
    return FPM_OK;
}

static int launch_fill(Compare &c, bool record_in)
{
    fpm_ctx *ctx = c.ctx;
    const DistFinal *fin = c.fin;
    PairFill fill;
    fill.dist = c.compact ? nullptr : fin->prim.dist;
    fill.pval = c.compact ? nullptr : fin->prim.pval;
    fill.pass = c.compact ? nullptr : fin->prim.pass;
    fill.max_dist = fin->par.max_dist;
    fill.max_pvalue = fin->par.max_pvalue;
    HIP_TRY(ensure_aux(ctx));
    if (record_in) HIP_TRY(hipEventRecord(ctx->ev_in, c.st));
    HIP_TRY(hipStreamWaitEvent(ctx->aux, ctx->ev_in, 0));
    TimedLaunch tl(ctx, FPM_K_FILL, ctx->aux);
    const long double cells_w = (long double)c.n_pairs * (c.want_mir ? 2 : 1);
    const bool flat = cells_w * 1.6L > (long double)ctx->last_events;
    HIP_TRY(launch_dist_fill(c.R.len, c.R.n, c.Q.len, c.Q.n, c.S, c.fill_cnt ? c.cnt : Counts{},
                             fill, ctx->aux, flat));
    if (c.want_mir) {
        PairFill mf = fill;
        mf.dist = c.compact ? nullptr : fin->mir.dist;
        mf.pval = c.compact ? nullptr : fin->mir.pval;
        mf.pass = c.compact ? nullptr : fin->mir.pass;
        HIP_TRY(launch_dist_fill(c.Q.len, c.Q.n, c.R.len, c.R.n, c.S, fin->mir.cnt, mf, ctx->aux,
                                 flat));
    }
    tl.done();
    HIP_TRY(hipEventRecord(ctx->ev_fill, ctx->aux));
    c.fill_pending = true;
    return FPM_OK;
}

static int index_transient(Compare &c, SparsePlan &p)
{
    fpm_ctx *ctx = c.ctx;
    hipStream_t st = c.st;
    const RowSet &R = c.R, &Q = c.Q;
    const uint32_t hash_bytes = c.hash_bytes;
    const bool self_set = c.self_set;
    unsigned long long *events = p.ctr;
    void *dir_, *entries_;
    HIP_TRY(scratch(ctx, kSlotDir, ((1ULL << p.geom.nbits) + 1) * 4, &dir_));
    HIP_TRY(scratch(ctx, kSlotEntries, (uint64_t)R.n * R.stride * 4, &entries_));
    p.dir = (const uint32_t *)dir_;
    p.entries = (const uint32_t *)entries_;
    auto count_probe = [&]() -> int {
        if (!self_set)
            HIP_TRY(launch_probe_count(p.p_rows, p.p_len ? p.p_len : Q.len, p.p_stride, Q.n,
                                       hash_bytes, p.geom, p.dir, events, p.unsorted(), st));
        return FPM_OK;
    };
    const uint64_t mr = std::min<uint64_t>(R.stride, c.S);
    const uint64_t mq = std::min<uint64_t>(Q.stride, c.S);
    void *dref = nullptr, *dref_len = nullptr, *dref_pos = nullptr, *dqry = nullptr,
         *dqry_len = nullptr, *dqry_pos = nullptr;
    auto records = [&](uint32_t *flag) -> int {
        HIP_TRY(scratch(ctx, kSlotRecRef, (size_t)R.n * mr * hash_bytes, &dref));
        HIP_TRY(scratch(ctx, kSlotRecRefLen, (size_t)R.n * 4, &dref_len));
        HIP_TRY(scratch(ctx, kSlotRecRefPos, (size_t)R.n * mr * 4, &dref_pos));
        if (!self_set) {
            HIP_TRY(scratch(ctx, kSlotRecQry, (size_t)Q.n * mq * hash_bytes, &dqry));
            HIP_TRY(scratch(ctx, kSlotRecQryLen, (size_t)Q.n * 4, &dqry_len));
            HIP_TRY(scratch(ctx, kSlotRecQryPos, (size_t)Q.n * mq * 4, &dqry_pos));
        }
        TimedLaunch tl(ctx, FPM_K_INDEX, st);
        HIP_TRY(launch_record_rows(R.rows, R.len, R.stride, R.n, hash_bytes, c.S, dref,
                                   (uint32_t *)dref_pos, (uint32_t *)dref_len, mr, st, flag));
        if (!self_set)
            HIP_TRY(launch_record_rows(Q.rows, Q.len, Q.stride, Q.n, hash_bytes, c.S, dqry,
                                       (uint32_t *)dqry_pos, (uint32_t *)dqry_len, mq, st, flag));
        tl.done();
        return FPM_OK;
    };
    auto record_index = [&]() -> int {
        p.rec_r = RecRows{dref, (const uint32_t *)dref_pos, (const uint32_t *)dref_len, mr};
        p.rec_q = self_set ? p.rec_r
                           : RecRows{dqry, (const uint32_t *)dqry_pos, (const uint32_t *)dqry_len, mq};
        p.p_rows = p.rec_q.val;
        p.p_len = p.rec_q.len;
        p.p_stride = p.rec_q.stride;
        p.geom = make_geom(R.n, (uint64_t)R.n * mr, 0);
        p.geom.kmax = events + kCtrKmax;
        if (int rc = build_index(ctx, RowSet{dref, p.rec_r.len, nullptr, mr, R.n}, hash_bytes,
                                 p.geom, (uint32_t *)dir_, (uint32_t *)entries_, events, self_set,
                                 st, count_probe, false, nullptr,
                                 c.list_zeroed ? nullptr : c.list_cnt))
            return rc;
        c.list_zeroed = true;
        p.all_sorted = false;
        p.ev = host_events(ctx);
        note_index(ctx, p.geom);
        return FPM_OK;
    };
    if (hash_bytes == 4) {
        HIP_TRY(hipMemsetAsync(p.unsorted(), 0, sizeof(uint32_t), st));
        if (int rc = records(p.unsorted())) return rc;
        if (int rc = read_counters(ctx, events, kCtrProbeWords, st)) return rc;
        if (host_unsorted(ctx)) return record_index();
    }
    p.geom.kmax = events + kCtrKmax;
    p.geom.vcut = index_cut_ok(c) ? 1u : 0u;
    const fpm_ctx::SpecProfile &pf = ctx->spec;
    const bool can_spec = pf.valid && hash_bytes == 8 && pf.n_ref == R.n && pf.n_qry == Q.n &&
                          pf.S == c.S && pf.ref_stride == R.stride && pf.qry_stride == Q.stride &&
                          pf.self_set == self_set && pf.defaults == c.probe_defaults() &&
                          ctx->dist_mode != FPM_DIST_DENSE && R.n <= (1u << 19) &&
                          std::max(R.stride, Q.stride) <= 2048;
    auto speculate = [&]() -> int {
        p.spec_probe = false;
        if (!can_spec) return FPM_OK;
        void *cand, *row_seg;
        HIP_TRY(scratch(ctx, kSlotCand, pf.cap * 8, &cand));
        HIP_TRY(scratch(ctx, kSlotRowSeg, (size_t)Q.n * 8, &row_seg));
        p.spec_half = probe_half(c, p, self_set);
        TimedLaunch tl(ctx, FPM_K_PROBE, st);
        HIP_TRY(launch_probe_rows(Q.rows, Q.len, Q.stride, Q.n, R.n, hash_bytes, p.geom, p.dir,
                                  p.entries, R.len, c.S, self_set, pf.defaults, self_set, c.cnt,
                                  (uint64_t *)cand, p.n_cand(), (uint64_t *)row_seg, nullptr,
                                  nullptr, nullptr, pf.cap, p.cand_over(), st, 0, p.spec_half));
        tl.done();
        p.spec_probe = true;
        return FPM_OK;
    };
    if (int rc = build_index(ctx, R, hash_bytes, p.geom, (uint32_t *)dir_, (uint32_t *)entries_,
                             events, self_set, st, count_probe, true, speculate,
                             c.list_zeroed ? nullptr : c.list_cnt))
        return rc;
    c.list_zeroed = true;
    p.ev = whole_index_events(host_events(ctx), host_entries(ctx), host_indexed(ctx));
    p.all_sorted = !host_unsorted(ctx);
    note_index(ctx, p.geom);
    if (p.all_sorted) return FPM_OK;
    if (hash_bytes != 4)
        if (int rc = records(nullptr)) return rc;
    return record_index();
}

static int index_phase(Compare &c, SparsePlan &p)
{
    fpm_ctx *ctx = c.ctx;
    fpm_refset *rs = c.rs;
    hipStream_t st = c.st;
    const RowSet &Q = c.Q;
    if (!rs) return index_transient(c, p);
    ctx->last_indexed = ctx->last_entries = rs->n_indexed;
    const long double ev_est =
        (long double)rs->self_events * Q.n / std::max<uint32_t>(1, rs->ref.n);
    p.skip_count = !c.self_set && !rs->recorded && !rs->ref_unsorted && c.hash_bytes == 8 &&
                   (ctx->dist_mode == FPM_DIST_SPARSE ||
                    (ctx->dist_mode == FPM_DIST_AUTO &&
                     ev_est * 16.0L <= (long double)c.n_pairs * c.S));
    p.geom = rs->geom;
    p.dir = rs->dir();
    p.entries = rs->entries();
    if (c.self_set && !rs->recorded) {
        p.ev = rs->self_events;
        p.all_sorted = !rs->ref_unsorted;
        HIP_TRY(hipMemsetAsync(p.ctr, 0, kCtrProbeWords * 8, st));
        return FPM_OK;
    }
    if (p.skip_count) {
        p.ev = (uint64_t)ev_est;
        p.all_sorted = true;
        HIP_TRY(hipMemsetAsync(p.ctr, 0, kCtrProbeWords * 8, st));
        return FPM_OK;
    }
    TimedLaunch tl(ctx, FPM_K_INDEX, st);
    HIP_TRY(hipMemsetAsync(p.ctr, 0, kCtrProbeWords * 8, st));
    if (rs->recorded) {
        const uint64_t mq = std::min<uint64_t>(Q.stride, c.S);
        void *dqry, *dqry_len, *dqry_pos;
        HIP_TRY(scratch(ctx, kSlotRecQry, (size_t)Q.n * mq * c.hash_bytes, &dqry));
        HIP_TRY(scratch(ctx, kSlotRecQryLen, (size_t)Q.n * 4, &dqry_len));
        HIP_TRY(scratch(ctx, kSlotRecQryPos, (size_t)Q.n * mq * 4, &dqry_pos));
        HIP_TRY(launch_record_rows(Q.rows, Q.len, Q.stride, Q.n, c.hash_bytes, c.S, dqry,
                                   (uint32_t *)dqry_pos, (uint32_t *)dqry_len, mq, st));
        p.rec_r = RecRows{rs->slot[fpm_refset::kRecRows].p,
                          (const uint32_t *)rs->slot[fpm_refset::kRecPos].p,
                          (const uint32_t *)rs->slot[fpm_refset::kRecLen].p, rs->mr};
        p.rec_q = RecRows{dqry, (const uint32_t *)dqry_pos, (const uint32_t *)dqry_len, mq};
        p.p_rows = dqry;
        p.p_len = (const uint32_t *)dqry_len;
        p.p_stride = mq;
    }
    HIP_TRY(launch_probe_count(p.p_rows, p.p_len ? p.p_len : Q.len, p.p_stride, Q.n,
                               c.hash_bytes, p.geom, p.dir, p.ctr, p.unsorted(), st));
    tl.done();
    if (int rc = read_counters(ctx, p.ctr, kCtrProbeWords, st)) return rc;
    p.ev = host_events(ctx);
    p.all_sorted = !rs->ref_unsorted && !rs->recorded && !host_unsorted(ctx);
    return FPM_OK;
}

static hipError_t rank_candidates(const Compare &c, const void *cand, const void *row_seg,
                                  bool sym, uint32_t *cnum, uint32_t *cden)
{
    uint32_t rank_cap = 0;
    const hipError_t e =
        launch_merge_rows((const uint64_t *)cand, (const uint64_t *)row_seg, c.Q.n,
                          (const uint64_t *)c.R.rows, c.R.len, c.R.stride, c.R.n,
                          (const uint64_t *)c.Q.rows, c.Q.len, c.Q.stride, c.S, sym, c.cnt, cnum,
                          cden, c.st, 0, &rank_cap);
    c.ctx->last_kernel = rank_cap == 1024 ? FPM_DK_CAND_RANK_1024 : FPM_DK_CAND_RANK_2048;
    return e;
}

static int candidate_phase(Compare &c, SparsePlan &p, bool rows_merge, uint64_t cap)
{
    fpm_ctx *ctx = c.ctx;
    hipStream_t st = c.st;
    const RowSet &R = c.R, &Q = c.Q;
    const DistFinal *fin = c.fin;
    const bool sym = rows_merge && c.self_set;
    const bool half = p.spec_probe ? p.spec_half : probe_half(c, p, sym);
    ctx->last_probe = half ? FPM_PROBE_HALF : FPM_PROBE_FULL;
    if (p.geom.vcut && !half) {
        p.geom.vcut = 0;
        p.spec_probe = false;
        if (int rc = build_index(ctx, R, c.hash_bytes, p.geom, const_cast<uint32_t *>(p.dir),
                                 const_cast<uint32_t *>(p.entries), p.ctr, c.self_set, st,
                                 [] { return FPM_OK; }))
            return rc;
        p.ev = host_events(ctx);
        note_index(ctx, p.geom);
        ctx->last_events = p.ev;
        cap = std::max<uint64_t>(1, std::min<uint64_t>(p.ev, c.n_pairs));
    }
    void *cand, *row_seg;
    HIP_TRY(scratch(ctx, kSlotCand, cap * 8, &cand));
    HIP_TRY(scratch(ctx, kSlotRowSeg, (size_t)Q.n * 8, &row_seg));
    if (!p.spec_probe) {
        TimedLaunch tl(ctx, FPM_K_PROBE, st);
        HIP_TRY(launch_probe_rows(p.p_rows, Q.len, p.p_stride, Q.n, R.n, c.hash_bytes, p.geom,
                                  p.dir, p.entries, R.len, c.S, sym, c.probe_defaults(),
                                  c.self_set, c.cnt, (uint64_t *)cand, p.n_cand(),
                                  (uint64_t *)row_seg, p.p_len,
                                  p.skip_count ? p.unsorted() : nullptr,
                                  p.skip_count ? p.ctr : nullptr, cap, p.cand_over(), st, 0,
                                  half));
        tl.done();
    }
    bool rank_done = false;
    if (p.skip_count) {
        unsigned long long seq;
        if (int rc = publish_counters(ctx, p.ctr, kCtrProbeWords, st, &seq)) return rc;
        if (fin && rows_merge) {
            void *cres;
            HIP_TRY(scratch(ctx, kSlotCandRes, cap * 8, &cres));
            if (c.need_fill) {
                HIP_TRY(ensure_aux(ctx));
                HIP_TRY(hipEventRecord(ctx->ev_in, st));
            }
            TimedLaunch tl(ctx, FPM_K_COMPARE, st);
            HIP_TRY(rank_candidates(c, cand, row_seg, sym, (uint32_t *)cres,
                                    (uint32_t *)cres + cap));
            tl.done();
            rank_done = true;
        }
        if (int rc = wait_counters(ctx, seq, st)) return rc;
        ctx->last_events = host_events(ctx);
        if (host_unsorted(ctx)) {
            p.all_sorted = false;
            rows_merge = false;
            rank_done = false;
        }
    }
    uint32_t *cnum = nullptr, *cden = nullptr;
    if (fin && rows_merge) {
        void *cres;
        HIP_TRY(scratch(ctx, kSlotCandRes, cap * 8, &cres));
        cnum = (uint32_t *)cres;
        cden = cnum + cap;
    }
    const bool defer_fill = c.need_fill && p.skip_count && rows_merge;
    if (defer_fill) {
        HIP_TRY(ensure_aux(ctx));
        if (!rank_done) HIP_TRY(hipEventRecord(ctx->ev_in, st));
    } else if (c.need_fill) {
        if (int rc = launch_fill(c, true)) return rc;
    }
    if (c.fill_pending && !cnum) HIP_TRY(hipStreamWaitEvent(st, ctx->ev_fill, 0));
    if (!cnum)
        if (int rc = settle_prefill(c)) return rc;
    if (!rank_done) {
        TimedLaunch tl(ctx, FPM_K_COMPARE, st);
        if (rows_merge)
            HIP_TRY(rank_candidates(c, cand, row_seg, sym, cnum, cden));
        else {
            HIP_TRY(launch_walk_candidates((const uint64_t *)cand, p.n_cand(), cap, R.rows, R.len,
                                           R.stride, R.n, Q.rows, Q.len, Q.stride, c.hash_bytes,
                                           c.S, c.cnt, p.rec_r, p.rec_q, st));
            ctx->last_kernel = FPM_DK_CAND_WALK;
        }
        tl.done();
    }
    if (defer_fill)
        if (int rc = launch_fill(c, false)) return rc;
    if (c.fill_pending && cnum) HIP_TRY(hipStreamWaitEvent(st, ctx->ev_fill, 0));
    if (int rc = settle_prefill(c)) return rc;
    if (fin) {
        if (int rc = zero_list(c)) return rc;
        const DistParams &par = fin->par;
        const bool mirror = c.want_mir && cnum;
        TimedLaunch tl(ctx, FPM_K_FINALIZE, st);
        if (c.compact) {
            const CellList none{};
            HIP_TRY(launch_dist_cand_list((const uint64_t *)cand, p.n_cand(), cap, sym, cnum, cden,
                                          c.cnt, R.length, Q.length, R.n, par.kmer_size,
                                          par.kmer_space, par.max_dist, par.max_pvalue,
                                          fin->prim.list, mirror ? fin->mir.cnt : Counts{}, Q.n,
                                          mirror ? fin->mir.list : none, st));
        } else {
            MirrorOut mir{};
            if (mirror) mir = MirrorOut{fin->mir.cnt, fin->mir.dist, fin->mir.pval, fin->mir.pass, Q.n};
            HIP_TRY(launch_dist_cand_finalize((const uint64_t *)cand, p.n_cand(), cap, sym, cnum,
                                              cden, c.cnt, R.length, Q.length, R.n, par.kmer_size,
                                              par.kmer_space, par.max_dist, par.max_pvalue,
                                              fin->prim.dist, fin->prim.pval, fin->prim.pass, mir,
                                              st));
        }
        tl.done();
        if (mirror && fin->mirrored) *fin->mirrored = true;
    }
    ctx->last_sparse = rows_merge ? 2 : 1;
    ctx->last_cand = (uint64_t)-1;
    ctx->last_cand_dev = p.n_cand();
    ctx->last_cand_stream = st;
    return FPM_OK;
}

static int dense_phase(Compare &c)
{
    fpm_ctx *ctx = c.ctx;
    hipStream_t st = c.st;
    const RowSet &R = c.R, &Q = c.Q;
    if (int rc = zero_list(c)) return rc;
    if (c.prefilled && !c.prefill_done) {
        HIP_TRY(hipStreamWaitEvent(st, ctx->ev_prefill, 0));
        c.prefill_done = true;
    }
    ctx->last_cand = c.n_pairs;
    void *ublk = nullptr, *bimg = nullptr;
    const bool img = compare_grid_img_ok(c.hash_bytes, c.S, R.stride, Q.stride);
    if (img) {
        size_t ub, bb;
        compare_grid_img_scratch(Q.n, c.S, R.stride, Q.stride, &ub, &bb);
        HIP_TRY(scratch(ctx, kSlotImgBlocks, ub, &ublk));
        HIP_TRY(scratch(ctx, kSlotImg, bb, &bimg));
    }
    TimedLaunch tl(ctx, FPM_K_COMPARE, st);
    if (img) {
        HIP_TRY(launch_compare_grid_img(R.rows, R.len, R.stride, R.n, Q.rows, Q.len, Q.stride,
                                        Q.n, c.S, ublk, bimg, c.cnt, st));
        ctx->last_kernel = FPM_DK_GRID_IMG;
    } else {
        bool lds = false;
        HIP_TRY(launch_compare_grid(R.rows, R.len, R.stride, R.n, Q.rows, Q.len, Q.stride, Q.n,
                                    c.hash_bytes, c.S, c.cnt, st, &lds));
        ctx->last_kernel = lds ? FPM_DK_GRID_LDS : FPM_DK_GRID_GLOBAL;
    }
    tl.done();
    return FPM_OK;
}

static int compare_impl(fpm_ctx *ctx, const RowSet &R, const RowSet &Q, uint32_t hash_bytes,
                        uint32_t sketch_size, Counts cnt, void *stream,
                        const DistFinal *fin = nullptr, bool *finalized = nullptr,
                        fpm_refset *rs = nullptr)
{
    if (finalized) *finalized = false;
    if (int rc = set_device(ctx)) return rc;
    if (hash_bytes != 4 && hash_bytes != 8) return fail(FPM_EINVAL, "hash_bytes must be 4 or 8");
    hipStream_t st = pick_stream(ctx, stream);
    if (ctx->prefill.pending) {
        HIP_TRY(hipStreamWaitEvent(st, ctx->ev_prefill, 0));
        ctx->prefill.pending = false;
    }
    const uint64_t n_pairs = (uint64_t)R.n * Q.n;
    ctx->last_sparse = 0;
    ctx->last_kernel = FPM_DK_NONE;
    ctx->last_probe = FPM_PROBE_NONE;
    ctx->last_index_cut = false;
    ctx->last_indexed = ctx->last_entries = 0;
    ctx->last_events = 0;
    ctx->last_cand = 0;
    if (n_pairs == 0) {
        if (fin && fin->compact()) HIP_TRY(hipMemsetAsync(fin->prim.list.count, 0, 8, st));
        return FPM_OK;
    }
    const uint64_t E = (uint64_t)R.n * R.stride;
    bool try_sparse = ctx->dist_mode == FPM_DIST_SPARSE ||
                      (ctx->dist_mode == FPM_DIST_AUTO && n_pairs >= 4096 && E > 0);
    if (E == 0) try_sparse = false;
    SparsePlan p;
    p.geom = make_geom(R.n, E, sketch_size);
    if (p.geom.rbits > 24 || E >= (1ULL << 31)) try_sparse = false;
    if (rs && !rs->sparse_ok) try_sparse = false;
    Compare c{ctx, st, R, Q, hash_bytes, sketch_size, cnt, fin, rs, n_pairs};
    c.self_set = R.rows == Q.rows && R.len == Q.len && R.stride == Q.stride && R.n == Q.n;
    c.compact = fin && fin->compact();
    c.want_mir = fin && fin->has_mirror() && !c.self_set;
    c.prefilled = fin && fin->prefilled;
    c.fill_cnt = fin && !c.prefilled &&
                 (c.want_mir || (ctx->fill_counts < 0 ? n_pairs >= (1ULL << 28)
                                                      : ctx->fill_counts != 0));
    c.need_fill = fin && (!c.compact || c.fill_cnt);
    c.list_cnt = c.compact ? reinterpret_cast<unsigned long long *>(fin->prim.list.count) : nullptr;
    c.list_zeroed = !c.compact;
    c.prefill_done = !c.prefilled;
    if (!try_sparse) return dense_phase(c);

    void *ctr;
    HIP_TRY(scratch(ctx, kSlotCounters, kCtrWords * 8, &ctr));
    p.ctr = (unsigned long long *)ctr;
    p.p_rows = Q.rows;
    p.p_stride = Q.stride;
    if (int rc = index_phase(c, p)) return rc;
    ctx->last_events = p.ev;
    const bool sparse = ctx->dist_mode == FPM_DIST_SPARSE ||
                        ((long double)p.ev * 4.0L <= (long double)n_pairs * sketch_size &&
                         (p.all_sorted || 2 * p.ev <= n_pairs));
    const bool rows_merge = sparse && p.all_sorted && hash_bytes == 8 && R.n <= (1u << 19) &&
                            std::max(R.stride, Q.stride) <= 2048;
    uint64_t cap = std::max<uint64_t>(1, p.skip_count ? n_pairs : std::min<uint64_t>(p.ev, n_pairs));
    if (p.spec_probe) {
        if (rows_merge && cap <= ctx->spec.cap) {
            cap = ctx->spec.cap;
            ctx->spec_hits++;
        } else {
            p.spec_probe = false;
            ctx->spec_misses++;
            HIP_TRY(hipMemsetAsync(p.n_cand(), 0, 8, st));
            HIP_TRY(hipMemsetAsync(p.cand_over(), 0, 4, st));
        }
    }
    if (rows_merge && !p.skip_count) {
        fpm_ctx::SpecProfile &pf = ctx->spec;
        const bool same = pf.valid && pf.n_ref == R.n && pf.n_qry == Q.n && pf.S == sketch_size &&
                          pf.ref_stride == R.stride && pf.qry_stride == Q.stride &&
                          pf.self_set == c.self_set;
        const uint64_t keep = same ? std::max(pf.cap, cap) : cap;
        pf = fpm_ctx::SpecProfile{true, R.n, Q.n, sketch_size, R.stride, Q.stride,
                                  keep, c.self_set, c.probe_defaults()};
    }
    if (!sparse) return dense_phase(c);
    if (int rc = candidate_phase(c, p, rows_merge, cap)) return rc;
    if (fin) *finalized = true;
    return FPM_OK;
}

static int dist_dev_impl(fpm_ctx *ctx, const RowSet &R, const RowSet &Q, uint32_t hash_bytes,
                         uint32_t sketch_size, const DistParams &par, const DistOut &out,
                         void *stream, const char *who, fpm_refset *rs = nullptr,
                         const DistOut *mirror = nullptr)
{
    const bool compact = out.list.count != nullptr;
    if (!R.length || !Q.length) return fail(FPM_EINVAL, std::string(who) + ": lengths required");
    if (!out.cnt.numer || !out.cnt.denom)
        return fail(FPM_EINVAL, std::string(who) + ": numer / denom buffers required");
    if (compact ? (!out.list.qry || !out.list.ref || !out.list.dist || !out.list.pval)
                : (!out.dist || !out.pval))
        return fail(FPM_EINVAL, std::string(who) +
                                    (compact ? ": list qry / ref / distance / p-value buffers required"
                                             : ": distance and p-value buffers required"));
    hipStream_t st = pick_stream(ctx, stream);
// ... 573 lines not shown
```

fp-mash_amd/csrc/fpm_internal.hpp:

```cpp
#pragma once

#include "fpm_kernels.hpp"
#include "../../include/fpmash.h"

#include <hip/hip_runtime.h>

#include <algorithm>
#include <condition_variable>
#include <cstdint>
#include <cstring>
#include <mutex>
#include <string>
#include <system_error>
#include <thread>
#include <vector>

using namespace fpm;

#define FPM_HIDDEN __attribute__((visibility("hidden")))

FPM_HIDDEN int fail(int code, const std::string &msg);

#define HIP_TRY(expr)                                                                      \
    do {                                                                                   \
// ... 14 lines not shown
        for (auto &t : th_) t.join();
    }
    void copy(void *dst, const void *src, size_t n)
    {
        constexpr size_t kPart = size_t(1) << 20;
        const unsigned want = (unsigned)std::min<size_t>(kMaxThreads + 1, n / kPart);
        if (want <= 1) { memcpy(dst, src, n); return; }
        std::unique_lock<std::mutex> lk(mu_);
        while (th_.size() + 1 < want && th_.size() < threads()) {
            try {
                th_.emplace_back([this] { work(); });
            } catch (const std::system_error &) {
                break;
            }
        }
        const unsigned parts = (unsigned)std::min<size_t>(want, th_.size() + 1);
        const size_t per = (n + parts - 1) / parts;
        char *d = static_cast<char *>(dst);
        const char *sp = static_cast<const char *>(src);
        for (unsigned i = 1; i < parts; i++) {
            const size_t a = i * per, b = std::min(n, a + per);
            if (a < b) { q_.push_back({d + a, sp + a, b - a}); pending_++; }
        }
        lk.unlock();
        cv_.notify_all();
        memcpy(d, sp, std::min(n, per));
        lk.lock();
        done_.wait(lk, [this] { return pending_ == 0; });
    }

  private:
    static constexpr unsigned kMaxThreads = 7;
    static unsigned threads()
    {
        const unsigned hw = std::max(1u, std::thread::hardware_concurrency());
        return std::min(kMaxThreads, std::max(1u, hw / 2));
    }
    struct Task { char *d; const char *s; size_t n; };
    void work()
    {
        std::unique_lock<std::mutex> lk(mu_);
        for (;;) {
            cv_.wait(lk, [this] { return stop_ || !q_.empty(); });
            if (q_.empty()) return;
            const Task t = q_.back();
            q_.pop_back();
            lk.unlock();
            memcpy(t.d, t.s, t.n);
            lk.lock();
            if (--pending_ == 0) done_.notify_all();
        }
    }
    std::mutex mu_;
    std::condition_variable cv_, done_;
    std::vector<std::thread> th_;
    std::vector<Task> q_;
    size_t pending_ = 0;
    bool stop_ = false;
};

enum ScratchSlot : int {
    kSlotTileHist = 0,
    kSlotTileOff = 1,
    kSlotTent = 2,
    kSlotCandRes = 3,
    kSlotDir = 4,
    kSlotEntries = 5,
    kSlotScan = 6,
    kSlotCounters = 7,
    kSlotCand = 8,
    kSlotRowSeg = 9,
    kSlotRecRef = 10,
    kSlotRecRefLen = 11,
    kSlotRecQry = 12,
    kSlotRecQryLen = 13,
    kSlotImgBlocks = 14,
    kSlotImg = 15,
    kSlotPartFill = 16,
    kSlotMergeRows = 16,
    kSlotMergeCounts = 17,
    kSlotMergeDescs = 18,
    kSlotRecRefPos = 19,
    kSlotRecQryPos = 20,
    kSlotCount
};

enum CtrWord : uint32_t {
    kCtrEvents = 0,
    kCtrPartials = 1,
    kCtrCand = 65,
    kCtrUnsorted = 66,
    kCtrOverflow = 67,
    kCtrIndexed = 68,
    kCtrEntries = 69,
    kCtrKmax = 70,
    kCtrCandOver = 71,
    kCtrKmaxAcc = 72,
    kCtrContain = 75,
    kCtrWords = 80,
    kCtrProbeWords = kCtrOverflow,
    kCtrBuildWords = kCtrKmax,
    kCtrZeroWords = kCtrKmaxAcc
};

struct fpm_ctx {
    int device = 0;
    hipStream_t stream = nullptr;
    bool timing = false;
    std::vector<std::pair<hipEvent_t, hipEvent_t>> ev[FPM_K_COUNT];
    struct Slot { void *p = nullptr; size_t bytes = 0; };
    Slot scratch[kSlotCount];
    unsigned long long *host_counters = nullptr;
    unsigned long long *dev_counters = nullptr;
    unsigned long long pub_seq = 0;
    int dist_mode = FPM_DIST_AUTO;
    int fill_counts = -1;
    int last_sparse = 0;
    int last_kernel = FPM_DK_NONE;
    bool probe_half = true;
    int last_probe = FPM_PROBE_NONE;
    bool index_cut = true;
    bool last_index_cut = false;
    uint64_t last_indexed = 0, last_entries = 0;
    int contain_mode = FPM_CONTAIN_AUTO;
    int last_contain_kernel = FPM_CK_NONE;
    int last_screen_kernel = FPM_SK_NONE;
    uint64_t last_events = 0, last_cand = 0;
    const unsigned long long *last_cand_dev = nullptr;
    hipStream_t last_cand_stream = nullptr;
    hipStream_t aux = nullptr;
    hipEvent_t ev_in = nullptr, ev_fill = nullptr;
    struct Prefill {
        const void *numer = nullptr, *denom = nullptr;
        uint32_t n_ref = 0, n_qry = 0, S = 0;
        bool pending = false;
    } prefill;
    hipEvent_t ev_prefill = nullptr;
    static constexpr int kRing = 4;
    static constexpr size_t kRingBytes = 8u << 20;
    void *ring[kRing] = {};
    hipEvent_t ring_ev[kRing] = {};
    CopyPool copier;
    static constexpr size_t kPoolBytes = size_t(2) << 30;
    uint64_t idx_rebuilds = 0;
    struct SpecProfile {
        bool valid = false;
        uint32_t n_ref = 0, n_qry = 0, S = 0;
        uint64_t ref_stride = 0, qry_stride = 0, cap = 0;
        bool self_set = false, defaults = false;
    } spec;
    uint64_t spec_hits = 0, spec_misses = 0;
    std::vector<std::pair<void *, size_t>> pool;
    size_t pool_bytes = 0;
    std::mutex pool_mu;
};

struct TimedLaunch {
    fpm_ctx *ctx; int kid; hipStream_t st; hipEvent_t a = nullptr, b = nullptr;
    TimedLaunch(fpm_ctx *c, int k, hipStream_t s) : ctx(c), kid(k), st(s)
    {
        if (ctx->timing) {
            (void)hipEventCreate(&a);
            (void)hipEventCreate(&b);
            (void)hipEventRecord(a, st);
        }
    }
    void done()
    {
        if (ctx->timing) {
            (void)hipEventRecord(b, st);
            ctx->ev[kid].push_back({a, b});
        }
    }
};

#pragma GCC visibility push(hidden)

int set_device(fpm_ctx *ctx);
inline hipStream_t pick_stream(fpm_ctx *ctx, void *stream)
{
    return stream ? (hipStream_t)stream : ctx->stream;
}

hipError_t pool_alloc(fpm_ctx *ctx, void **p, size_t bytes);
void pool_free(fpm_ctx *ctx, void *p, size_t bytes);

hipError_t ensure_ring(fpm_ctx *ctx);
hipError_t memset_sync(fpm_ctx *ctx, void *dst, int v, size_t bytes);
hipError_t h2d_staged(fpm_ctx *ctx, void *dst, const void *src, size_t bytes);
hipError_t d2h_staged(fpm_ctx *ctx, void *dst, const void *src, size_t bytes);
hipError_t copy_out(fpm_ctx *ctx, void *dst, const void *src, size_t bytes);
hipError_t copy_in(fpm_ctx *ctx, void *dst, const void *src, size_t bytes);
hipError_t ensure_aux(fpm_ctx *ctx);

hipError_t grow_slot(fpm_ctx::Slot &s, size_t bytes, void **out);
hipError_t scratch(fpm_ctx *ctx, ScratchSlot id, size_t bytes, void **out);

int publish_counters(fpm_ctx *ctx, const unsigned long long *d_src, uint32_t n, hipStream_t st,
                     unsigned long long *seq_out);
int wait_counters(fpm_ctx *ctx, unsigned long long seq, hipStream_t st);
int read_counters(fpm_ctx *ctx, const unsigned long long *d_src, uint32_t n, hipStream_t st);

inline uint64_t host_events(const fpm_ctx *ctx) { return ctx->host_counters[kCtrEvents]; }
inline bool host_flag(const fpm_ctx *ctx, CtrWord w)
{
    return ((const uint32_t *)(ctx->host_counters + w))[0] != 0;
// ... 34 lines not shown
```

fp-mash_amd/csrc/fpm_kernels.hpp:

```cpp
#pragma once

#include <hip/hip_runtime.h>
#include <stdint.h>

namespace fpm {

struct TileDesc {
    uint64_t byte_off;
    uint32_t n_bytes;
    uint32_t out_row;
    uint32_t thr_slot;
    uint32_t pad;
};

struct SketchKParams {
    uint32_t k;
    uint32_t s;
    uint32_t seed;
    uint32_t use64;
    uint32_t canonical;
    uint32_t preserve_case;
    uint32_t compl_acgt;
    uint8_t alphabet[256];
    uint8_t complement[256];
// ... 67 lines not shown
hipError_t launch_merge(const MergeDesc *d_desc, uint32_t n, uint32_t s, bool small,
                        hipStream_t st);

hipError_t launch_fp_hash(const uint64_t *d_vals, const uint64_t *d_line_off, uint64_t n_lines,
                          uint32_t seed, uint32_t use64, void *d_out, hipStream_t st);

hipError_t launch_compare_grid(const void *d_ref, const uint32_t *d_ref_len, uint64_t ref_stride,
                               uint32_t n_ref, const void *d_qry, const uint32_t *d_qry_len,
                               uint64_t qry_stride, uint32_t n_qry, uint32_t hash_bytes,
                               uint32_t sketch_size, Counts cnt, hipStream_t st,
                               bool *lds = nullptr);

bool compare_grid_img_ok(uint32_t hash_bytes, uint32_t sketch_size, uint64_t ref_stride,
                         uint64_t qry_stride);
void compare_grid_img_scratch(uint32_t n_qry, uint32_t sketch_size, uint64_t ref_stride,
                              uint64_t qry_stride, size_t *ublk_bytes, size_t *bimg_bytes);
hipError_t launch_compare_grid_img(const void *d_ref, const uint32_t *d_ref_len,
                                   uint64_t ref_stride, uint32_t n_ref, const void *d_qry,
                                   const uint32_t *d_qry_len, uint64_t qry_stride, uint32_t n_qry,
                                   uint32_t sketch_size, void *ublk, void *bimg, Counts cnt,
                                   hipStream_t st);
struct RecRows {
    const void *val = nullptr;
    const uint32_t *pos = nullptr, *len = nullptr;
    uint64_t stride = 0;
};
hipError_t launch_walk_candidates(const uint64_t *d_cand, const unsigned long long *d_n_cand,
                                  uint64_t cap, const void *d_ref, const uint32_t *d_ref_len,
                                  uint64_t ref_stride, uint32_t n_ref, const void *d_qry,
                                  const uint32_t *d_qry_len, uint64_t qry_stride,
                                  uint32_t hash_bytes, uint32_t S, Counts cnt, RecRows rec_ref,
                                  RecRows rec_qry, hipStream_t st);

constexpr uint32_t kIdxL1 = 10;
constexpr uint32_t kIdxTile = 16384;
struct IdxGeom {
    uint32_t l2;
    uint32_t nbits;
    uint32_t rbits;
    uint32_t fbits;
    uint32_t ntiles;
    uint32_t tile;
    const unsigned long long *kmax;
    uint32_t cap;
    uint32_t cut;
    uint32_t vcut;
};
uint64_t idx_tent_words(const IdxGeom &g, uint64_t E);
hipError_t launch_idx_build(const void *d_ref, const uint32_t *d_ref_len, uint64_t stride,
                            uint32_t n_ref, uint32_t hash_bytes, IdxGeom g, uint32_t *tile_hist,
                            uint32_t *tile_off, uint32_t *scan_s, uint64_t *tent,
                            uint32_t *dir, uint32_t *entries, uint32_t *unsorted,
                            unsigned long long *self_events, unsigned long long *zero,
                            uint32_t nzero, unsigned long long *acc, uint32_t *part_fill,
                            uint32_t *overflow, hipStream_t st,
                            unsigned long long *zero_x = nullptr,
                            unsigned long long *n_entries = nullptr);
uint64_t scan_scratch_words(uint64_t n);
constexpr uint32_t kPubWords = 128;
hipError_t launch_publish(const unsigned long long *d_src, uint32_t n, unsigned long long *h_dst,
                          unsigned long long seq, hipStream_t st);
hipError_t launch_record_rows(const void *in, const uint32_t *in_len, uint64_t in_stride,
                              uint32_t n, uint32_t hash_bytes, uint32_t S, void *out,
                              uint32_t *pos_out, uint32_t *out_len, uint64_t out_stride,
                              hipStream_t st, uint32_t *unsorted = nullptr);
hipError_t launch_exscan(const uint32_t *in, uint32_t *out, uint32_t *out2, uint64_t n,
                         uint32_t *scratch, uint32_t *total, hipStream_t st);
hipError_t launch_probe_count(const void *d_qry, const uint32_t *d_qry_len, uint64_t stride,
                              uint32_t n_qry, uint32_t hash_bytes, IdxGeom g, const uint32_t *dir,
                              unsigned long long *events, uint32_t *unsorted, hipStream_t st);
struct PairFill {
    double *dist = nullptr, *pval = nullptr;
    uint8_t *pass = nullptr;
    double max_dist = -1, max_pvalue = -1;
};
hipError_t launch_dist_fill(const uint32_t *d_ref_len, uint32_t n_ref, const uint32_t *d_qry_len,
                            uint32_t n_qry, uint32_t S, Counts cnt, const PairFill &fill,
                            hipStream_t st, bool flat = true);
hipError_t launch_dist_counts_const(uint16_t *numer, uint16_t *denom, uint64_t cells, uint32_t S,
                                    hipStream_t st);
hipError_t launch_dist_counts_fixup(const uint32_t *d_ref_len, uint32_t n_ref,
                                    const uint32_t *d_qry_len, uint32_t n_qry, uint32_t S,
                                    uint16_t *denom, hipStream_t st);
hipError_t launch_probe_rows(const void *d_qry, const uint32_t *d_qry_len, uint64_t stride,
                             uint32_t n_qry, uint32_t n_ref, uint32_t hash_bytes, IdxGeom g,
                             const uint32_t *dir, const uint32_t *entries,
                             const uint32_t *d_ref_len, uint32_t S, bool sym, bool defaults,
                             bool self_set, Counts cnt, uint64_t *cand,
                             unsigned long long *n_cand, uint64_t *row_seg,
                             const uint32_t *d_qry_it_len, uint32_t *q_unsorted,
                             unsigned long long *events, uint64_t cap, uint32_t *cand_over,
                             hipStream_t st, uint32_t q_lo = 0, bool half = false);
hipError_t launch_merge_rows(const uint64_t *d_cand, const uint64_t *row_seg, uint32_t n_qry,
                             const uint64_t *d_ref, const uint32_t *d_ref_len, uint64_t ref_stride,
                             uint32_t n_ref, const uint64_t *d_qry, const uint32_t *d_qry_len,
                             uint64_t qry_stride, uint32_t S, bool sym, Counts cnt,
                             uint32_t *d_cnum, uint32_t *d_cden, hipStream_t st, uint32_t q_lo = 0,
                             uint32_t *rank_cap = nullptr);

uint32_t text_blocks(uint64_t len);
uint32_t fp_text_chunk();
uint32_t fp_span_bytes();
uint32_t fp_head_lines();
hipError_t launch_fp_nl_count(const uint8_t *d_text, uint64_t len, uint32_t *blk_cnt,
                              uint32_t *blk_off, uint32_t *scan_s, hipStream_t st);
hipError_t launch_fp_nl_scatter(const uint8_t *d_text, uint64_t len, const uint32_t *blk_off,
                                uint64_t *d_line_start, hipStream_t st);
uint32_t fp_head_blocks(uint64_t n_lines);
hipError_t launch_fp_heads(const uint8_t *d_new_id, uint64_t n_lines, uint32_t *blk_cnt,
                           uint32_t *blk_off, uint32_t *scan_s, hipStream_t st);
hipError_t launch_fp_refs(const uint8_t *d_new_id, uint64_t n_lines, const uint32_t *blk_off,
                          uint64_t n_refs, const uint32_t *d_n_vals, const uint64_t *d_id_off,
                          const uint32_t *d_id_len, uint64_t *d_first, uint64_t *d_length,
                          uint64_t *d_ref_id_off, uint32_t *d_ref_id_len, hipStream_t st);
hipError_t launch_fp_lines(const uint8_t *d_text, uint64_t len, const uint64_t *d_line_start,
                           uint64_t n_nl, uint64_t n_lines, uint32_t seed, uint32_t use64,
                           uint64_t *id_off, uint32_t *id_len, uint32_t *n_vals, void *hash,
                           uint8_t *new_id, hipStream_t st);

constexpr uint32_t kSpChunk = 4096;
size_t seq_xf_bytes();
size_t seq_cin_bytes();
hipError_t launch_seq_scan(const uint8_t *d_text, const uint8_t *d_reset, uint32_t n_chunks,
                           void *d_xf, void *d_cin, uint64_t *d_totals, hipStream_t st);
hipError_t launch_seq_emit(const uint8_t *d_text, uint32_t n_chunks, const void *d_cin,
                           uint64_t n_rec, uint64_t total_kept, uint64_t *d_hdr_pos,
                           uint64_t *d_hdr_end, uint64_t *d_kept_at, uint64_t *d_seq_off,
                           uint64_t *d_seq_len, uint8_t *d_out, hipStream_t st);

hipError_t launch_fq_files(const uint64_t *d_line_start, uint64_t n_starts, const uint64_t *d_seg,
                           uint32_t n_seg, uint64_t *d_file_lines, hipStream_t st);
hipError_t launch_fq_records(const uint8_t *d_text, const uint64_t *d_line_start,
                             const uint64_t *d_seg, const uint64_t *d_file_lines,
                             const uint64_t *d_rec_base, uint32_t n_seg, uint64_t n_rec,
                             uint64_t *d_rec, uint64_t *d_scan, uint64_t *d_total, uint32_t *d_fail,
                             uint8_t *d_out, hipStream_t st);
hipError_t launch_fq_emit(const uint8_t *d_text, uint64_t n_rec, uint64_t *d_rec, uint8_t *d_out,
                          hipStream_t st);

hipError_t launch_positional_grid(const void *d_ref, const uint32_t *d_ref_len,
                                  uint64_t ref_stride, uint32_t n_ref, const void *d_qry,
                                  const uint32_t *d_qry_len, uint64_t qry_stride, uint32_t n_qry,
                                  uint32_t hash_bytes, double max_dist, double max_pvalue,
                                  uint32_t *d_numer, uint32_t *d_denom, double *d_dist,
                                  double *d_pvalue, uint8_t *d_pass, hipStream_t st);

hipError_t launch_rows_ascending(const void *d_ref, const uint32_t *d_ref_len, uint64_t ref_stride,
                                 uint32_t n_ref, const void *d_qry, const uint32_t *d_qry_len,
                                 uint64_t qry_stride, uint32_t n_qry, uint32_t hash_bytes,
                                 uint32_t *flag, hipStream_t st);
uint32_t contain_lds_cap(uint32_t hash_bytes);
hipError_t launch_contain_rows(const void *d_ref, const uint32_t *d_ref_len, uint64_t ref_stride,
                               uint32_t n_ref, const void *d_qry, const uint32_t *d_qry_len,
                               uint64_t qry_stride, uint32_t n_qry, uint32_t hash_bytes,
                               uint32_t max_qry_len, uint32_t *d_common, uint32_t *d_steps,
                               hipStream_t st, bool *lds);
hipError_t launch_contain_literal(const void *d_ref, const uint32_t *d_ref_len,
                                  uint64_t ref_stride, uint32_t n_ref, const void *d_qry,
                                  const uint32_t *d_qry_len, uint64_t qry_stride, uint32_t n_qry,
                                  uint32_t hash_bytes, uint32_t *d_common, uint32_t *d_steps,
                                  hipStream_t st);

struct ScreenTable;
constexpr uint32_t kScreenRowsLdsCap = 12288;
hipError_t launch_screen_sort(const void *d_db, const uint32_t *d_len, uint64_t stride,
                              uint32_t n_db, uint32_t hash_bytes, uint32_t E, uint32_t sbits,
                              unsigned long long *kmax, uint32_t *hist, uint32_t *start,
                              uint32_t *scan_s, uint64_t *skey, uint32_t *scell, uint64_t *okey,
                              uint32_t *ocell, hipStream_t st);
hipError_t launch_screen_heads(const uint64_t *okey, uint32_t E, uint32_t *head, uint32_t *hx,
                               uint32_t *scan_s, uint32_t *n_distinct, hipStream_t st);
hipError_t launch_screen_compact(const uint64_t *okey, const uint32_t *ocell, const uint32_t *head,
                                 const uint32_t *hx, uint32_t E, uint64_t stride, uint32_t n,
                                 uint32_t dbits, uint32_t shift, uint64_t *U, uint32_t *ustart,
                                 uint32_t *slot, uint32_t *post, uint32_t *dir, hipStream_t st);
hipError_t launch_screen_count(int cls, const uint8_t *d_seq, const TileDesc *d_tiles,
                               uint32_t n_tiles, const SketchKParams &p, const ScreenTable &t,
                               hipStream_t st);
hipError_t launch_screen_hashes(const uint64_t *d_keys, uint64_t n, const ScreenTable &t,
                                hipStream_t st);
hipError_t launch_screen_rows(const uint32_t *d_slot, const uint32_t *d_len, uint64_t stride,
// ... 54 lines not shown
```

fp-mash_amd/fpmash/__init__.py:

```python
from __future__ import annotations

import ctypes as C
import os

import numpy as np

PKG_ROOT = os.path.dirname(os.path.dirname(os.path.abspath(__file__)))
LIB_PATH = os.environ.get("FPMASH_LIB") or os.path.join(PKG_ROOT, "lib", "libfpmash.so")
BIN_PATH = os.path.join(PKG_ROOT, "bin", "fpmash")

FPM_OK, FPM_EINVAL, FPM_ENODEV, FPM_EHIP, FPM_ENOMEM = 0, -1, -2, -3, -4
(K_SKETCH, K_MERGE, K_FPHASH, K_COMPARE, K_FINALIZE, K_INDEX, K_PROBE, K_FPTEXT, K_FILL,
 K_SEQPARSE, K_SCREEN) = range(11)
NO_GROUP = 0xFFFFFFFF
KERNEL_NAMES = {K_SKETCH: "sketch_tiles_kernel", K_MERGE: "merge_kernel",
                K_FPHASH: "fp_hash_kernel",
                K_COMPARE: "candidate compare (rank_rows/walk_cand/compare_grid), contain_rows/contain_literal",
                K_FINALIZE: "dist finalize (dense / candidate cells)", K_INDEX: "dist index build",
                K_PROBE: "probe_rows_kernel", K_FPTEXT: "fp text parse (nl index + fp_line)",
                K_FILL: "dist_fill_kernel", K_SEQPARSE: "FASTA parse (seq chunk scan + emit)",
                K_SCREEN: "screen_count_kernel"}
DIST_AUTO, DIST_DENSE, DIST_SPARSE = 0, 1, 2
DIST_PATHS = ["dense walk", "bucket index + literal walk", "bucket index + bucketed rank"]
(DK_NONE, DK_GRID_GLOBAL, DK_GRID_LDS, DK_GRID_IMG, DK_CAND_WALK, DK_CAND_RANK_1024,
 DK_CAND_RANK_2048) = range(7)
DIST_KERNELS = ["none", "compare_grid_kernel", "compare_grid_lds_kernel",
                "compare_grid_img_kernel", "walk_cand_kernel", "rank_rows_kernel<1024>",
                "rank_rows_kernel<2048>"]
PROBE_NONE, PROBE_FULL, PROBE_HALF = range(3)
CONTAIN_AUTO, CONTAIN_LITERAL = range(2)
CK_NONE, CK_ROWS_LDS, CK_ROWS_GLOBAL, CK_LITERAL = range(4)
CONTAIN_KERNELS = ["none", "contain_rows_kernel<lds>", "contain_rows_kernel<global>",
                   "contain_literal_kernel"]
CONTAIN_BLOCK_REFS = 64
SK_NONE, SK_ROWS_LDS, SK_ROWS_GLOBAL = range(3)
SCREEN_KERNELS = ["none", "screen_rows_kernel<lds>", "screen_rows_kernel<global>"]

ALPHABET_NUCLEOTIDE = "ACGT"
ALPHABET_PROTEIN = "ACDEFGHIKLMNPQRSTVWY"

u64p = C.POINTER(C.c_uint64)
u32p = C.POINTER(C.c_uint32)
f64p = C.POINTER(C.c_double)
u8p = C.POINTER(C.c_uint8)
vp = C.c_void_p

SYMBOLS = [
    ("fpm_abi_version", C.c_int, []),
    ("fpm_build_id", C.c_char_p, []),
    ("fpm_last_error", C.c_char_p, []),
    ("fpm_device_count", C.c_int, [C.POINTER(C.c_int)]),
    ("fpm_ctx_create", C.c_int, [C.c_int, C.POINTER(vp)]),
    ("fpm_ctx_destroy", None, [vp]),
    ("fpm_ctx_stream", vp, [vp]),
    ("fpm_stream_create", C.c_int, [vp, C.POINTER(vp)]),
    ("fpm_stream_destroy", C.c_int, [vp, vp]),
    ("fpm_event_create", C.c_int, [vp, C.POINTER(vp)]),
    ("fpm_event_destroy", C.c_int, [vp, vp]),
    ("fpm_event_record", C.c_int, [vp, vp, vp]),
    ("fpm_stream_wait_event", C.c_int, [vp, vp, vp]),
    ("fpm_ctx_synchronize", C.c_int, [vp]),
    ("fpm_ctx_warm", C.c_int, [vp]),
    ("fpm_malloc", C.c_int, [vp, C.POINTER(vp), C.c_size_t]),
    ("fpm_free", C.c_int, [vp, vp]),
    ("fpm_memcpy_h2d", C.c_int, [vp, vp, vp, C.c_size_t]),
    ("fpm_memcpy_d2h", C.c_int, [vp, vp, vp, C.c_size_t]),
    ("fpm_memcpy_d2d", C.c_int, [vp, vp, vp, C.c_size_t]),
    ("fpm_memset", C.c_int, [vp, vp, C.c_int, C.c_size_t]),
    ("fpm_ctx_set_timing", C.c_int, [vp, C.c_int]),
    ("fpm_ctx_reset_timing", C.c_int, [vp]),
    ("fpm_ctx_kernel_time", C.c_int, [vp, C.c_int, f64p, u64p]),
    ("fpm_ctx_set_dist_mode", C.c_int, [vp, C.c_int]),
    ("fpm_ctx_last_dist_stats", C.c_int, [vp, C.POINTER(C.c_int), u64p, u64p]),
    ("fpm_ctx_last_dist_kernel", C.c_int, [vp, C.POINTER(C.c_int)]),
    ("fpm_ctx_set_probe_half", C.c_int, [vp, C.c_int]),
    ("fpm_ctx_last_dist_probe", C.c_int, [vp, C.POINTER(C.c_int)]),
    ("fpm_ctx_set_index_cut", C.c_int, [vp, C.c_int]),
    ("fpm_ctx_last_index_cut", C.c_int, [vp, C.POINTER(C.c_int), u64p, u64p]),
    ("fpm_sketch_batch", C.c_int, [vp, vp, C.c_char_p, u64p, C.c_uint32, u32p, C.c_uint32,
                                   u64p, u32p]),
    ("fpm_sketch_stage", C.c_int, [vp, vp, C.c_char_p, u64p, C.c_uint32, u32p, C.c_uint32,
                                   C.POINTER(vp)]),
    ("fpm_sketch_run", C.c_int, [vp, vp]),
    ("fpm_sketch_device_output", C.c_int, [vp, C.POINTER(vp), C.POINTER(vp), u32p, u32p]),
    ("fpm_sketch_fetch", C.c_int, [vp, u64p, u32p]),
    ("fpm_sketch_mult", C.c_int, [vp, vp, u32p]),
    ("fpm_sketch_job_set_min_copies", C.c_int, [vp, C.c_uint32]),
    ("fpm_sketch_reads_run", C.c_int, [vp, vp]),
    ("fpm_sketch_reads_fetch", C.c_int, [vp, u64p, u32p, u32p, u64p]),
    ("fpm_sketch_job_reads_rounds", C.c_int, [vp, C.POINTER(C.c_int32), u32p]),
    ("fpm_sketch_job_reads_sampled", C.c_int, [vp, C.POINTER(C.c_int32)]),
    ("fpm_merge_small_spills", C.c_int, [vp, u64p]),
    ("fpm_sketch_job_info", C.c_int, [vp, u64p, u64p, u64p]),
    ("fpm_sketch_job_redo_tiles", C.c_int, [vp, C.POINTER(C.c_int32)]),
    ("fpm_sketch_job_short_groups", C.c_int, [vp, C.POINTER(C.c_int32)]),
    ("fpm_sketch_job_sample_short", C.c_int, [vp, C.POINTER(C.c_int32)]),
    ("fpm_sketch_job_plan", C.c_int, [vp, vp]),
    ("fpm_sketch_job_free", None, [vp]),
    ("fpm_fp_hash_lines", C.c_int, [vp, u64p, u64p, C.c_uint64, C.c_uint32, C.c_uint32, vp]),
    ("fpm_fp_hash_lines_dev", C.c_int, [vp, vp, vp, C.c_uint64, C.c_uint32, C.c_uint32, vp,
                                        vp]),
    ("fpm_fp_text_stage", C.c_int, [vp, C.c_char_p, C.c_uint64, C.c_uint64, C.c_uint32,
                                    C.c_uint32, C.POINTER(vp), u64p]),
    ("fpm_fp_text_fetch", C.c_int, [vp, u64p, u32p, u32p, vp, u8p]),
    ("fpm_fp_text_refs", C.c_int, [vp, C.c_uint64, u64p, u64p, u64p, u32p, u64p]),
    ("fpm_fp_text_free", None, [vp]),
    ("fpm_fp_text_limits", None, [u32p, u32p, u32p]),
    ("fpm_compare_grid", C.c_int, [vp, vp, u32p, C.c_uint64, C.c_uint32, vp, u32p, C.c_uint64,
                                   C.c_uint32, C.c_uint32, C.c_uint32, u32p, u32p]),
    ("fpm_compare_grid_dev", C.c_int, [vp, vp, vp, C.c_uint64, C.c_uint32, vp, vp, C.c_uint64,
                                       C.c_uint32, C.c_uint32, C.c_uint32, vp, vp, vp]),
    ("fpm_dist_finalize_dev", C.c_int, [vp, vp, vp, vp, vp, C.c_uint32, C.c_uint32, C.c_uint32,
                                        C.c_double, C.c_double, C.c_double, vp, vp, vp, vp]),
    ("fpm_pvalue_batch_dev", C.c_int, [vp, vp, vp, C.c_uint32, vp, vp, C.c_uint64, C.c_uint32,
                                       C.c_double, vp, vp, vp]),
    ("fpm_dist_dev", C.c_int, [vp, vp, vp, vp, C.c_uint64, C.c_uint32, vp, vp, vp, C.c_uint64,
                               C.c_uint32, C.c_uint32, C.c_uint32, C.c_uint32, C.c_double,
                               C.c_double, C.c_double, vp, vp, vp, vp, vp, vp]),
    ("fpm_dist_dev16", C.c_int, [vp, vp, vp, vp, C.c_uint64, C.c_uint32, vp, vp, vp, C.c_uint64,
                                 C.c_uint32, C.c_uint32, C.c_uint32, C.c_uint32, C.c_double,
                                 C.c_double, C.c_double, vp, vp, vp, vp, vp, vp]),
    ("fpm_dist_list_dev", C.c_int, [vp, vp, vp, vp, C.c_uint64, C.c_uint32, vp, vp, vp,
                                    C.c_uint64, C.c_uint32, C.c_uint32, C.c_uint32, C.c_uint32,
                                    C.c_double, C.c_double, C.c_double, vp, vp, vp, vp]),
    ("fpm_dist_list_prefill", C.c_int, [vp, vp, vp, C.c_uint32, C.c_uint32, C.c_uint32, vp]),
    ("fpm_fp_positional_grid", C.c_int, [vp, vp, u32p, C.c_uint64, C.c_uint32, vp, u32p,
                                         C.c_uint64, C.c_uint32, C.c_uint32, C.c_double,
                                         C.c_double, u32p, u32p, f64p, f64p, u8p]),
    ("fpm_dist", C.c_int, [vp, vp, u32p, u64p, C.c_uint64, C.c_uint32, vp, u32p, u64p,
                           C.c_uint64, C.c_uint32, C.c_uint32, C.c_uint32, C.c_uint32,
                           C.c_double, C.c_double, C.c_double, u32p, u32p, f64p, f64p, u8p]),
    ("fpm_contain", C.c_int, [vp, vp, u32p, C.c_uint64, C.c_uint32, vp, u32p, C.c_uint64,
                              C.c_uint32, C.c_uint32, u32p, u32p]),
    ("fpm_contain_dev", C.c_int, [vp, vp, vp, C.c_uint64, C.c_uint32, vp, vp, C.c_uint64,
                                  C.c_uint32, C.c_uint32, vp, vp, vp]),
    ("fpm_ctx_set_contain_mode", C.c_int, [vp, C.c_int]),
    ("fpm_ctx_last_contain_kernel", C.c_int, [vp, C.POINTER(C.c_int)]),
    ("fpm_contain_lds_cap", C.c_int, [vp, C.c_uint32, u32p]),
    ("fpm_screen_create", C.c_int, [vp, vp, u32p, C.c_uint64, C.c_uint32, C.c_uint32,
                                    C.c_uint32, C.POINTER(vp)]),
    ("fpm_screen_create_dev", C.c_int, [vp, vp, vp, C.c_uint64, C.c_uint32, C.c_uint32,
                                        C.c_uint32, C.POINTER(vp)]),
    ("fpm_screen_free", None, [vp]),
    ("fpm_screen_add_job", C.c_int, [vp, vp, vp]),
    ("fpm_screen_add_hashes_dev", C.c_int, [vp, vp, C.c_uint64, vp]),
    ("fpm_screen_set_size", C.c_int, [vp, u64p]),
    ("fpm_screen_counts", C.c_int, [vp, u64p, u32p, u64p]),
    ("fpm_screen_rows", C.c_int, [vp, u32p, u32p]),
    ("fpm_screen_rows_winner", C.c_int, [vp, f64p, u64p, u32p, u32p]),
    ("fpm_screen_pvalues", C.c_int, [vp, u32p, C.c_double, f64p]),
    ("fpm_ctx_last_screen_kernel", C.c_int, [vp, C.POINTER(C.c_int)]),
    ("fpm_screen_lds_cap", C.c_int, [vp, u32p]),
    ("fpm_refset_create", C.c_int, [vp, vp, u32p, u64p, C.c_uint64, C.c_uint32, C.c_uint32,
                                    C.c_uint32, C.POINTER(vp)]),
    ("fpm_refset_create_dev", C.c_int, [vp, vp, vp, vp, C.c_uint64, C.c_uint32, C.c_uint32,
                                        C.c_uint32, C.POINTER(vp)]),
    ("fpm_refset_dist_dev", C.c_int, [vp, vp, vp, vp, C.c_uint64, C.c_uint32, C.c_uint32,
                                      C.c_uint32, C.c_uint32, C.c_double, C.c_double, C.c_double,
                                      vp, vp, vp, vp, vp, vp]),
    ("fpm_refset_dist_mirror_dev", C.c_int, [vp, vp, vp, vp, C.c_uint64, C.c_uint32, C.c_uint32,
                                             C.c_uint32, C.c_uint32, C.c_double, C.c_double,
# ... 494 lines not shown
    def stream(self):
        return lib().fpm_ctx_stream(self.h)

    def synchronize(self):
        _check(lib().fpm_ctx_synchronize(self.h))

    def new_stream(self):
        s = vp()
        _check(lib().fpm_stream_create(self.h, C.byref(s)))
        return s.value

    def free_stream(self, s):
        _check(lib().fpm_stream_destroy(self.h, s))

    def new_event(self):
        e = vp()
        _check(lib().fpm_event_create(self.h, C.byref(e)))
        return e.value

    def free_event(self, e):
        _check(lib().fpm_event_destroy(self.h, e))

    def record(self, event, stream):
        _check(lib().fpm_event_record(self.h, event, stream))

    def wait(self, stream, event):
        _check(lib().fpm_stream_wait_event(self.h, stream, event))

    def set_timing(self, on=True):
        _check(lib().fpm_ctx_set_timing(self.h, int(on)))

    def reset_timing(self):
        _check(lib().fpm_ctx_reset_timing(self.h))

    def kernel_time(self, kernel):
        t, n = C.c_double(), C.c_uint64()
        _check(lib().fpm_ctx_kernel_time(self.h, kernel, C.byref(t), C.byref(n)))
        return t.value, n.value

    def merge_small_spills(self):
        v = np.zeros(1, np.uint64)
        _check(lib().fpm_merge_small_spills(self.h, _p(v, u64p)))
        return int(v[0])

    def set_dist_mode(self, mode):
        _check(lib().fpm_ctx_set_dist_mode(self.h, mode))

    def index_rebuilds(self):
        v = C.c_uint64()
        _check(lib().fpm_ctx_index_rebuilds(self.h, C.byref(v)))
        return v.value

    def spec_stats(self):
        h, m = C.c_uint64(), C.c_uint64()
        _check(lib().fpm_ctx_spec_stats(self.h, C.byref(h), C.byref(m)))
        return h.value, m.value

    def last_dist_stats(self):
        sp, ev, ca = C.c_int(), C.c_uint64(), C.c_uint64()
        _check(lib().fpm_ctx_last_dist_stats(self.h, C.byref(sp), C.byref(ev), C.byref(ca)))
        return {"sparse": sp.value, "events": ev.value, "candidates": ca.value}

    def last_dist_kernel(self):
        k = C.c_int()
        _check(lib().fpm_ctx_last_dist_kernel(self.h, C.byref(k)))
        return k.value

    def set_probe_half(self, on=True):
        _check(lib().fpm_ctx_set_probe_half(self.h, int(on)))

    def last_dist_probe(self):
        f = C.c_int()
        _check(lib().fpm_ctx_last_dist_probe(self.h, C.byref(f)))
        return f.value

    def set_index_cut(self, on=True):
        _check(lib().fpm_ctx_set_index_cut(self.h, int(on)))

    def last_index_cut(self):
        c, i, e = C.c_int(), C.c_uint64(), C.c_uint64()
        _check(lib().fpm_ctx_last_index_cut(self.h, C.byref(c), C.byref(i), C.byref(e)))
        return {"cut": bool(c.value), "indexed": i.value, "entries": e.value}

    def sketch(self, params, seqs, groups=None, n_groups=None, counts=False, min_copies=1):
        if min_copies != 1:
            r = self.sketch_reads(params, seqs, groups, n_groups, min_copies)
            return (r["hashes"], r["counts"]) if counts else r["hashes"]
        job = SketchJob(self, params, seqs, groups, n_groups)
        try:
            job.run()
            rows, cnt = job.fetch()
            mult = job.mult() if counts else None
        finally:
            job.free()
        hashes = [rows[i, : cnt[i]].copy() for i in range(len(cnt))]
        if counts:
            return hashes, [mult[i, : cnt[i]].copy() for i in range(len(cnt))]
        return hashes

    def sketch_job(self, params, seqs, groups=None, n_groups=None, min_copies=1):
        return SketchJob(self, params, seqs, groups, n_groups, min_copies)

    @staticmethod
    def _reads_result(job):
        job.run_reads()
        rows, cnt, mult, est = job.fetch_reads()
        rounds, per = job.reads_rounds()
        return {"hashes": [rows[i, : cnt[i]].copy() for i in range(len(cnt))],
                "counts": [mult[i, : cnt[i]].copy() for i in range(len(cnt))],
                "estimate": est.copy(), "rounds": rounds, "group_round": per,
                "sampled": job.reads_sampled()}

    def sketch_reads(self, params, seqs, groups=None, n_groups=None, min_copies=1):
        job = SketchJob(self, params, seqs, groups, n_groups, min_copies)
        try:
            return self._reads_result(job)
        finally:
            job.free()

    def seq_parse(self, files):
        n_seg = len(files)
        ptrs = (C.c_char_p * max(n_seg, 1))(*files)
        lens = np.array([len(f) for f in files] + [0], dtype=np.uint64)
        job, n, q = vp(), C.c_uint64(), C.c_int()
        _check(lib().fpm_seq_parse(self.h, ptrs, _p(lens, u64p), n_seg, C.byref(job),
                                   C.byref(n), C.byref(q)))
        n = n.value
        seg = np.zeros(max(n, 1), np.uint32)
        ho, hl, sl = (np.zeros(max(n, 1), np.uint64) for _ in range(3))
        try:
            _check(lib().fpm_seq_records(job, _p(seg, u32p), _p(ho, u64p), _p(hl, u64p),
                                         _p(sl, u64p)))
        except Exception:
            lib().fpm_seq_free(job)
            raise
        return job.value, {"seg": seg[:n], "hdr_off": ho[:n], "hdr_len": hl[:n],
                           "seq_len": sl[:n]}, bool(q.value)

    def seq_packed(self, seq_job, n_rec=None, cap=None):
        nb = C.c_uint64()
        _check(lib().fpm_seq_packed(seq_job, None, None, 0, C.byref(nb)))
        size = nb.value if cap is None else cap
        out = np.zeros(max(size, 1), np.uint8)
        off = np.zeros(max(nb.value, 1), np.uint64)
        _check(lib().fpm_seq_packed(seq_job, _p(off, u64p), _p(out, u8p), size, C.byref(nb)))
        if n_rec is None:
            n_rec = int(np.count_nonzero(out[:nb.value] == 0))
        return out[:nb.value].tobytes(), off[:n_rec].copy()

    def sketch_seq_job(self, params, seq_job, groups, n_groups):
        g = np.ascontiguousarray(groups, dtype=np.uint32)
        if g.size == 0:
            g = np.zeros(1, np.uint32)
        h = vp()
        _check(lib().fpm_sketch_stage_seq(self.h, C.byref(params), seq_job, _p(g, u32p),
                                          n_groups, C.byref(h)))
        job = SketchJob.__new__(SketchJob)
        job.ctx, job.params, job.n_groups, job.h, job._keep = self, params, n_groups, h.value, None
        return job

    def sketch_seq(self, params, seq_job, groups, n_groups, counts=False, min_copies=1):
        job = self.sketch_seq_job(params, seq_job, groups, n_groups)
        if min_copies != 1:
            try:
                job.set_min_copies(min_copies)
                r = self._reads_result(job)
# ... 362 lines not shown
```

include/fpmash.h:

```cpp
#ifndef FPMASH_H
#define FPMASH_H

#include <stddef.h>
#include <stdint.h>

#ifdef __cplusplus
extern "C" {
#endif

#define FPM_OK 0
#define FPM_EINVAL (-1)
#define FPM_ENODEV (-2)
#define FPM_EHIP (-3)
#define FPM_ENOMEM (-4)

#define FPM_ABI_VERSION 1

typedef struct fpm_ctx fpm_ctx;
typedef struct fpm_sketch_job fpm_sketch_job;

typedef struct fpm_sketch_params {
    uint32_t kmer_size;
    uint32_t sketch_size;
    uint32_t seed;
    uint32_t use64;
    uint32_t noncanonical;
    uint32_t preserve_case;
    uint8_t alphabet[256];
} fpm_sketch_params;

int fpm_abi_version(void);
const char *fpm_build_id(void);
const char *fpm_last_error(void);
int fpm_device_count(int *count);
int fpm_ctx_create(int device, fpm_ctx **out);
void fpm_ctx_destroy(fpm_ctx *ctx);
void *fpm_ctx_stream(fpm_ctx *ctx);
int fpm_ctx_synchronize(fpm_ctx *ctx);
int fpm_stream_create(fpm_ctx *ctx, void **stream);
int fpm_stream_destroy(fpm_ctx *ctx, void *stream);
int fpm_event_create(fpm_ctx *ctx, void **event);
int fpm_event_destroy(fpm_ctx *ctx, void *event);
int fpm_event_record(fpm_ctx *ctx, void *event, void *stream);
int fpm_stream_wait_event(fpm_ctx *ctx, void *stream, void *event);
int fpm_ctx_warm(fpm_ctx *ctx);

int fpm_malloc(fpm_ctx *ctx, void **dptr, size_t bytes);
int fpm_free(fpm_ctx *ctx, void *dptr);
int fpm_memcpy_h2d(fpm_ctx *ctx, void *dst, const void *src, size_t bytes);
int fpm_memcpy_d2h(fpm_ctx *ctx, void *dst, const void *src, size_t bytes);
int fpm_memcpy_d2d(fpm_ctx *ctx, void *dst, const void *src, size_t bytes);
int fpm_memset(fpm_ctx *ctx, void *dptr, int value, size_t bytes);

#define FPM_K_SKETCH 0
#define FPM_K_MERGE 1
#define FPM_K_FPHASH 2
#define FPM_K_COMPARE 3
#define FPM_K_FINALIZE 4
#define FPM_K_INDEX 5
#define FPM_K_PROBE 6
#define FPM_K_FPTEXT 7
#define FPM_K_FILL 8
#define FPM_K_SEQPARSE 9
#define FPM_K_SCREEN 10
#define FPM_K_COUNT 11
int fpm_ctx_index_rebuilds(fpm_ctx *ctx, uint64_t *count);
int fpm_ctx_spec_stats(fpm_ctx *ctx, uint64_t *hits, uint64_t *misses);
int fpm_ctx_set_timing(fpm_ctx *ctx, int enable);
int fpm_ctx_reset_timing(fpm_ctx *ctx);
int fpm_ctx_kernel_time(fpm_ctx *ctx, int kernel, double *total_ms, uint64_t *launches);
int fpm_merge_small_spills(fpm_ctx *ctx, uint64_t *count);

#define FPM_DIST_AUTO 0
#define FPM_DIST_DENSE 1
#define FPM_DIST_SPARSE 2
int fpm_ctx_set_dist_mode(fpm_ctx *ctx, int mode);
int fpm_ctx_last_dist_stats(fpm_ctx *ctx, int *sparse, uint64_t *events, uint64_t *candidates);
#define FPM_DK_NONE 0
#define FPM_DK_GRID_GLOBAL 1
#define FPM_DK_GRID_LDS 2
#define FPM_DK_GRID_IMG 3
#define FPM_DK_CAND_WALK 4
#define FPM_DK_CAND_RANK_1024 5
#define FPM_DK_CAND_RANK_2048 6
int fpm_ctx_last_dist_kernel(fpm_ctx *ctx, int *kernel);
int fpm_ctx_set_probe_half(fpm_ctx *ctx, int on);
#define FPM_PROBE_NONE 0
#define FPM_PROBE_FULL 1
#define FPM_PROBE_HALF 2
int fpm_ctx_last_dist_probe(fpm_ctx *ctx, int *form);
int fpm_ctx_set_index_cut(fpm_ctx *ctx, int on);
int fpm_ctx_last_index_cut(fpm_ctx *ctx, int *cut, uint64_t *indexed, uint64_t *entries);

int fpm_sketch_batch(fpm_ctx *ctx, const fpm_sketch_params *p, const char *seq,
                     const uint64_t *rec_off, uint32_t n_rec, const uint32_t *group_of_rec,
                     uint32_t n_groups, uint64_t *out_hashes, uint32_t *out_count);

int fpm_sketch_stage(fpm_ctx *ctx, const fpm_sketch_params *p, const char *seq,
                     const uint64_t *rec_off, uint32_t n_rec, const uint32_t *group_of_rec,
                     uint32_t n_groups, fpm_sketch_job **job);
int fpm_sketch_run(fpm_sketch_job *job, void *stream);
int fpm_sketch_device_output(fpm_sketch_job *job, uint64_t **d_hashes, uint32_t **d_count,
                             uint32_t *n_groups, uint32_t *row_stride);
int fpm_sketch_fetch(fpm_sketch_job *job, uint64_t *out_hashes, uint32_t *out_count);
int fpm_sketch_mult(fpm_sketch_job *job, void *stream, uint32_t *out_mult);
int fpm_sketch_job_set_min_copies(fpm_sketch_job *job, uint32_t min_copies);
int fpm_sketch_reads_run(fpm_sketch_job *job, void *stream);
int fpm_sketch_reads_fetch(fpm_sketch_job *job, uint64_t *out_hashes, uint32_t *out_count,
                           uint32_t *out_mult, uint64_t *out_estimate);
int fpm_sketch_job_reads_rounds(fpm_sketch_job *job, int32_t *n_rounds, uint32_t *group_round);
int fpm_sketch_job_reads_sampled(fpm_sketch_job *job, int32_t *n_sampled);
int fpm_sketch_job_info(fpm_sketch_job *job, uint64_t *seq_bytes, uint64_t *n_tiles,
                        uint64_t *n_kmers);
int fpm_sketch_job_redo_tiles(fpm_sketch_job *job, int32_t *n_redo);
int fpm_sketch_job_short_groups(fpm_sketch_job *job, int32_t *n_short);
int fpm_sketch_job_sample_short(fpm_sketch_job *job, int32_t *n_short);
#define FPM_TILE_CLASSES 6
#define FPM_MK_LDS 0
#define FPM_MK_GLOBAL 1
typedef struct fpm_sketch_plan {
    uint32_t tiles[FPM_TILE_CLASSES];
    uint32_t sample_tiles[FPM_TILE_CLASSES];
    uint32_t thr4;
    uint32_t n_slots;
    uint32_t tight;
    uint32_t n_ssel, n_sel;
    uint32_t rounds, rounds_small;
    uint32_t sample_rounds, sample_rounds_small;
    uint32_t merge_kernel;
} fpm_sketch_plan;
int fpm_sketch_job_plan(fpm_sketch_job *job, fpm_sketch_plan *out);
void fpm_sketch_job_free(fpm_sketch_job *job);

int fpm_sketch_merge_dev(fpm_ctx *ctx, const uint64_t *d_lists, const uint32_t *d_counts,
                         uint32_t n_lists, uint32_t s, uint64_t *d_out, uint32_t *d_out_count,
                         void *stream);

typedef struct fpm_seqtext fpm_seqtext;
#define FPM_NO_GROUP 0xFFFFFFFFu
int fpm_seq_parse(fpm_ctx *ctx, const char *const *seg_text, const uint64_t *seg_len,
                  uint32_t n_seg, fpm_seqtext **job, uint64_t *n_records, int *quality_lines);
int fpm_seq_records(fpm_seqtext *job, uint32_t *seg_of_rec, uint64_t *hdr_off, uint64_t *hdr_len,
                    uint64_t *seq_len);
int fpm_seq_packed(fpm_seqtext *job, uint64_t *seq_off, uint8_t *out, uint64_t cap,
                   uint64_t *n_bytes);
int fpm_sketch_stage_seq(fpm_ctx *ctx, const fpm_sketch_params *p, fpm_seqtext *seq,
                         const uint32_t *group_of_rec, uint32_t n_groups, fpm_sketch_job **job);
void fpm_seq_free(fpm_seqtext *job);

int fpm_fp_hash_lines(fpm_ctx *ctx, const uint64_t *vals, const uint64_t *line_off,
                      uint64_t n_lines, uint32_t seed, uint32_t use64, void *out);
int fpm_fp_hash_lines_dev(fpm_ctx *ctx, const uint64_t *d_vals, const uint64_t *d_line_off,
                          uint64_t n_lines, uint32_t seed, uint32_t use64, void *d_out,
                          void *stream);

typedef struct fpm_fptext fpm_fptext;
int fpm_fp_text_stage(fpm_ctx *ctx, const char *text, uint64_t text_len, uint64_t max_lines,
                      uint32_t seed, uint32_t use64, fpm_fptext **job, uint64_t *n_lines);
int fpm_fp_text_fetch(fpm_fptext *job, uint64_t *id_off, uint32_t *id_len, uint32_t *n_vals,
                      void *hash, uint8_t *new_id);
int fpm_fp_text_refs(fpm_fptext *job, uint64_t cap, uint64_t *n_refs, uint64_t *first_line,
                     uint64_t *id_off, uint32_t *id_len, uint64_t *length);
void fpm_fp_text_free(fpm_fptext *job);
void fpm_fp_text_limits(uint32_t *text_chunk, uint32_t *span_bytes, uint32_t *head_lines);

int fpm_compare_grid(fpm_ctx *ctx, const void *ref, const uint32_t *ref_len,
                     uint64_t ref_stride, uint32_t n_ref, const void *qry,
                     const uint32_t *qry_len, uint64_t qry_stride, uint32_t n_qry,
                     uint32_t hash_bytes, uint32_t sketch_size, uint32_t *out_numer,
                     uint32_t *out_denom);
int fpm_compare_grid_dev(fpm_ctx *ctx, const void *d_ref, const uint32_t *d_ref_len,
                         uint64_t ref_stride, uint32_t n_ref, const void *d_qry,
                         const uint32_t *d_qry_len, uint64_t qry_stride, uint32_t n_qry,
                         uint32_t hash_bytes, uint32_t sketch_size, uint32_t *d_numer,
                         uint32_t *d_denom, void *stream);
// ... 159 lines not shown
```

Baseline: 26.18 billion bases/s.

## Compact reference rows to probe-hit entries before rank merge in symmetric half probe

During the half-probe index pass, the probe kernel records which of each row's first half entries hit any other row, and writes a compacted copy of the row: kept hashes plus their original positions as 16-bit values. The rank kernel then streams only these compacted rows and uses the stored positions to compute union ranks, so it loads and probes fewer entries per pair. The cost is an extra compacted-row buffer, extra LDS and ballot work in the probe kernel, and extra per-lane position loads in the rank kernel. Self pairs are special-cased. The path only applies to symmetric all-vs-all comparisons with rows up to 2048 entries.

```diff
diff --git a/fp-mash_amd/csrc/dist.hip b/fp-mash_amd/csrc/dist.hip
--- a/fp-mash_amd/csrc/dist.hip
+++ b/fp-mash_amd/csrc/dist.hip
@@ -8,6 +8,7 @@
 #include <float.h>
 
 #include <algorithm>
+#include <type_traits>
 
 namespace fpm {
 
@@ -281,14 +282,14 @@
     }
 }
 
-template <int CAP, typename C>
+template <int CAP, typename C, bool CMP = false>
 __global__ __launch_bounds__(64 * kRankWaves) void rank_rows_kernel(
     const uint64_t *__restrict__ cand, const uint64_t *__restrict__ row_seg, uint32_t n_qry,
     uint32_t q_lo, const uint64_t *__restrict__ ref, const uint32_t *__restrict__ ref_len,
     uint64_t ref_stride, uint32_t n_ref, const uint64_t *__restrict__ qry,
     const uint32_t *__restrict__ qry_len, uint64_t qry_stride, uint32_t S, uint32_t sym,
     C *__restrict__ numer, C *__restrict__ denom, uint32_t *__restrict__ cnum,
-    uint32_t *__restrict__ cden)
+    uint32_t *__restrict__ cden, CmpRows cm)
 {
     constexpr uint32_t kLogBuckets = (CAP <= 1024) ? kRankLogB : kRankLogB + 1;
     constexpr uint32_t kBuckets = 1u << kLogBuckets;
@@ -369,21 +370,26 @@
     const uint64_t pair_row = (uint64_t)q * n_ref;
     constexpr int kGroup = 1;
     constexpr uint32_t kChunk = 128;
-    struct Row { __amdgpu_buffer_rsrc_t rsrc; uint32_t la; uint64_t o; };
+    struct Row { __amdgpu_buffer_rsrc_t rsrc; uint32_t la, lc; uint64_t o; };
+    const uint32_t row_bytes = CMP ? (uint32_t)cmp_row_bytes(ref_stride) : ld * 8u;
     auto open_row = [&](uint64_t o) -> Row {
         const uint32_t rr = __builtin_amdgcn_readfirstlane((uint32_t)(o - pair_row));
-        const uintptr_t Ar = (uintptr_t)(ref + (uint64_t)rr * ref_stride);
+        const uintptr_t Ar = CMP ? (uintptr_t)cm.rows + (uint64_t)rr * row_bytes
+                                 : (uintptr_t)(ref + (uint64_t)rr * ref_stride);
         const uint32_t plo = __builtin_amdgcn_readfirstlane((uint32_t)Ar);
         const uint32_t phi = __builtin_amdgcn_readfirstlane((uint32_t)(Ar >> 32));
         Row R;
         R.rsrc = __builtin_amdgcn_make_buffer_rsrc((void *)(((uintptr_t)phi << 32) | plo), 0,
-                                                   (int)__builtin_amdgcn_readfirstlane(ld * 8u),
+                                                   (int)__builtin_amdgcn_readfirstlane(row_bytes),
                                                    0x00020000);
         R.la = ref_len[rr];
+        R.lc = CMP ? (rr == q ? 0u : cm.len[rr]) : R.la;
         R.o = o;
         return R;
     };
-    struct Pair { uint64_t e0, e1; };
+    struct PairV { uint64_t e0, e1; };
+    struct PairP { uint64_t e0, e1; uint32_t pp; };
+    using Pair = std::conditional_t<CMP, PairP, PairV>;
     auto load_group = [&](const Row &R, uint32_t gi, Pair (&dst)[kGroup]) {
 #pragma unroll
         for (int u = 0; u < kGroup; u++) {
@@ -393,6 +399,9 @@
                                                                  0, 0);
             dst[u].e0 = ((uint64_t)v0[1] << 32) | v0[0];
             dst[u].e1 = ((uint64_t)v1[1] << 32) | v1[0];
+            if constexpr (CMP)
+                dst[u].pp = __builtin_amdgcn_raw_buffer_load_b32(R.rsrc, (t * 64 + lane) * 4u,
+                                                                 (int)(ld * 8u), 0);
         }
     };
     auto cand_at = [&](uint32_t cc) -> uint64_t {
@@ -404,13 +413,22 @@
         uint32_t j0, j1;
         const uint64_t m0 = probe(cur[0].e0, j0);
         const uint64_t m1 = probe(cur[0].e1, j1);
-        const uint32_t i0 = g0 * kChunk;
+        uint32_t i0l, i1l, i_last;
+        if constexpr (CMP) {
+            i0l = cur[0].pp & 0xFFFFu;
+            i1l = cur[0].pp >> 16;
+            i_last = last ? 0u : (uint32_t)__builtin_amdgcn_readlane((int)cur[0].pp, 63) >> 16;
+        } else {
+            i0l = g0 * kChunk + lane;
+            i1l = i0l + 64;
+            i_last = g0 * kChunk + (kChunk - 1);
+        }
         const uint64_t a0 = m0 & vm0, a1 = m1 & vm1;
         const uint32_t p0 = (uint32_t)__popcll(a0), p1 = (uint32_t)__popcll(a1);
         uint32_t u_last = 0;
         if (!last) {
             const uint32_t jl = (uint32_t)__builtin_amdgcn_readlane((int)j1, 63);
-            u_last = i0 + (kChunk - 1) + jl -
+            u_last = i_last + jl -
                      (shared_below + p0 + (uint32_t)__popcll(a1 & 0x7FFFFFFFFFFFFFFFULL));
         }
         if (!last && u_last < S) {
@@ -422,7 +440,7 @@
                 (uint32_t)(a1 >> 32), __builtin_amdgcn_mbcnt_lo((uint32_t)a1, 0u));
             const uint32_t k0 = shared_below + b0;
             const uint32_t k1 = shared_below + p0 + b1;
-            const uint32_t u0 = i0 + lane + j0 - k0, u1 = i0 + 64 + lane + j1 - k1;
+            const uint32_t u0 = i0l + j0 - k0, u1 = i1l + j1 - k1;
             cnt += __popcll(a0 & __builtin_amdgcn_ballot_w64(u0 < S)) +
                    __popcll(a1 & __builtin_amdgcn_ballot_w64(u1 < S));
         }
@@ -441,10 +459,11 @@
             const uint32_t la = R.la;
             const uint64_t o = R.o;
             const bool need_all = la < S && lb < S;
-            const uint32_t nch = (la + kChunk - 1) / kChunk;
+            const uint32_t ls = R.lc;
+            const uint32_t nch = (ls + kChunk - 1) / kChunk;
             const uint32_t ngr = (nch + kGroup - 1) / kGroup;
             static_assert(kGroup == 1, "the last-chunk masks assume one chunk per group");
-            const int rl = (int)la - (int)(nch - 1) * (int)kChunk;
+            const int rl = (int)ls - (int)(nch - 1) * (int)kChunk;
             const int r0 = min(rl, 64), r1 = rl - 64;
             const uint64_t vl0 = r0 >= 64 ? ~0ULL : r0 > 0 ? (1ULL << r0) - 1 : 0ULL;
             const uint64_t vl1 = r1 >= 64 ? ~0ULL : r1 > 0 ? (1ULL << r1) - 1 : 0ULL;
@@ -464,6 +483,9 @@
                 const uint64_t x0 = fast ? __builtin_amdgcn_ballot_w64(cur[0].e0 == ~0ULL) : 0;
                 const uint64_t x1 = fast ? __builtin_amdgcn_ballot_w64(cur[0].e1 == ~0ULL) : 0;
                 rank_group(probe, gi * kGroup, true, vl0 & ~x0, vl1 & ~x1, cur, shared_below, cnt);
+            }
+            if constexpr (CMP) {
+                if ((uint32_t)(o - pair_row) == q) { shared_below = lb; cnt = lb < S ? lb : S; }
             }
             if (lane == 0) {
                 const uint64_t un = (uint64_t)la + lb - shared_below;
@@ -508,19 +530,33 @@
                                const uint32_t *d_qry_len, uint64_t qry_stride, uint32_t S,
                                bool sym, C *d_numer, C *d_denom, uint32_t *d_cnum,
                                uint32_t *d_cden, hipStream_t st, uint32_t q_lo,
-                               uint32_t *rank_cap)
+                               uint32_t *rank_cap, CmpRows cmp)
 {
     const dim3 g(xcd_grid(n_qry)), b(64 * kRankWaves);
     const uint64_t cap = std::max(ref_stride, qry_stride);
     if (rank_cap) *rank_cap = cap <= 1024 ? 1024u : 2048u;
+    if (cmp.rows) {
+        if (!cmp.len || !sym || d_ref != d_qry || ref_stride != qry_stride || q_lo != 0 ||
+            n_qry != n_ref || cap > 2048)
+            return hipErrorInvalidValue;
+        if (cap <= 1024)
+            hipLaunchKernelGGL((rank_rows_kernel<1024, C, true>), g, b, 0, st, d_cand, row_seg,
+                               n_qry, q_lo, d_ref, d_ref_len, ref_stride, n_ref, d_qry, d_qry_len,
+                               qry_stride, S, (uint32_t)sym, d_numer, d_denom, d_cnum, d_cden, cmp);
+        else
+            hipLaunchKernelGGL((rank_rows_kernel<2048, C, true>), g, b, 0, st, d_cand, row_seg,
+                               n_qry, q_lo, d_ref, d_ref_len, ref_stride, n_ref, d_qry, d_qry_len,
+                               qry_stride, S, (uint32_t)sym, d_numer, d_denom, d_cnum, d_cden, cmp);
+        return hipGetLastError();
+    }
     if (cap <= 1024)
         hipLaunchKernelGGL((rank_rows_kernel<1024, C>), g, b, 0, st, d_cand, row_seg, n_qry, q_lo,
                            d_ref, d_ref_len, ref_stride, n_ref, d_qry, d_qry_len, qry_stride, S,
-                           (uint32_t)sym, d_numer, d_denom, d_cnum, d_cden);
+                           (uint32_t)sym, d_numer, d_denom, d_cnum, d_cden, cmp);
     else if (cap <= 2048)
         hipLaunchKernelGGL((rank_rows_kernel<2048, C>), g, b, 0, st, d_cand, row_seg, n_qry, q_lo,
                            d_ref, d_ref_len, ref_stride, n_ref, d_qry, d_qry_len, qry_stride, S,
-                           (uint32_t)sym, d_numer, d_denom, d_cnum, d_cden);
+                           (uint32_t)sym, d_numer, d_denom, d_cnum, d_cden, cmp);
     else
         return hipErrorInvalidValue;
     return hipGetLastError();
@@ -531,16 +567,16 @@
                              uint32_t n_ref, const uint64_t *d_qry, const uint32_t *d_qry_len,
                              uint64_t qry_stride, uint32_t S, bool sym, Counts cnt,
                              uint32_t *d_cnum, uint32_t *d_cden, hipStream_t st, uint32_t q_lo,
-                             uint32_t *rank_cap)
+                             uint32_t *rank_cap, CmpRows cmp)
 {
     if (!n_qry) return hipSuccess;
     if (cnt.c16)
         return merge_rows_c(d_cand, row_seg, n_qry, d_ref, d_ref_len, ref_stride, n_ref, d_qry,
                             d_qry_len, qry_stride, S, sym, (uint16_t *)cnt.numer,
-                            (uint16_t *)cnt.denom, d_cnum, d_cden, st, q_lo, rank_cap);
+                            (uint16_t *)cnt.denom, d_cnum, d_cden, st, q_lo, rank_cap, cmp);
     return merge_rows_c(d_cand, row_seg, n_qry, d_ref, d_ref_len, ref_stride, n_ref, d_qry,
                         d_qry_len, qry_stride, S, sym, (uint32_t *)cnt.numer,
-                        (uint32_t *)cnt.denom, d_cnum, d_cden, st, q_lo, rank_cap);
+                        (uint32_t *)cnt.denom, d_cnum, d_cden, st, q_lo, rank_cap, cmp);
 }
 
 
diff --git a/fp-mash_amd/csrc/dist_index.hip b/fp-mash_amd/csrc/dist_index.hip
--- a/fp-mash_amd/csrc/dist_index.hip
+++ b/fp-mash_amd/csrc/dist_index.hip
@@ -607,7 +607,7 @@
     if (threadIdx.x == 0) events[0] = v;
 }
 
-template <typename C, bool HALF>
+template <typename C, bool HALF, bool CMP = false>
 __global__ __launch_bounds__(256) __attribute__((amdgpu_waves_per_eu(8)))
 void probe_rows_kernel(
     const void *__restrict__ qry, const uint32_t *__restrict__ qry_len, uint64_t stride,
@@ -618,14 +618,21 @@
     C *__restrict__ denom, uint64_t *__restrict__ cand,
     unsigned long long *__restrict__ n_cand, uint64_t *__restrict__ row_seg,
     const uint32_t *__restrict__ qry_it_len, uint32_t *__restrict__ q_unsorted,
-    unsigned long long *__restrict__ events, uint64_t cap, uint32_t *__restrict__ cand_over)
-{
+    unsigned long long *__restrict__ events, uint64_t cap, uint32_t *__restrict__ cand_over,
+    CmpRows cm)
+{
+    static_assert(!CMP || HALF, "the compacted rows are the half probe's");
     extern __shared__ __attribute__((aligned(16))) uint32_t rowbits[];
     __shared__ uint32_t wsum[4];
     __shared__ unsigned long long row_base;
+    constexpr uint32_t kKeepWords = CMP ? kCmpMaxRow / 32 : 1;
+    __shared__ __attribute__((aligned(8))) uint32_t s_keep[kKeepWords];
+    __shared__ uint32_t s_kpre[CMP ? 64 : 1];
+    __shared__ uint32_t s_kept;
     constexpr uint32_t kWin = 1024;
     __shared__ uint64_t w_tab[4][64];
     __shared__ uint8_t w_own[4][kWin];
+    __shared__ uint64_t w_hit[4][CMP ? kWin / 64 : 1];
     const uint32_t qr = xcd_row(blockIdx.x, n_qry);
     if (qr >= n_qry) return;
     const uint32_t q = q_lo + qr;
@@ -642,6 +649,8 @@
     const uint32_t nwords = (r1 - r0 + 31) / 32;
     const uint32_t both0 = nwords * 32;
     for (uint32_t w = threadIdx.x; w < nwords * (HALF ? 2 : 1); w += 256) rowbits[w] = 0;
+    if constexpr (CMP)
+        if (threadIdx.x < kKeepWords) s_keep[threadIdx.x] = 0;
     __syncthreads();
     const uint32_t lq = qry_len[q];
     const uint32_t lit = HALF ? (lq >= S ? (S + 1) / 2 : lq) : qry_it_len ? qry_it_len[q] : lq;
@@ -685,6 +694,7 @@
         ev_w += total;
         const uint32_t pre = inc - cnt;
         w_tab[wave][lane] = ((uint64_t)tgt << 32) | (uint32_t)(st - pre);
+        bool keptl = false;
         for (uint32_t wb = 0; wb < total; wb += kWin) {
             const uint32_t a0 = max(pre, wb), a1 = min(pre + cnt, wb + kWin);
             for (uint32_t e = a0; e < a1; e++) w_own[wave][e - wb] = (uint8_t)lane;
@@ -711,11 +721,14 @@
                     const uint32_t r = en[u] & rmask;
                     const bool hit = e < wn &&
                                      ((en[u] & ~kEntryFlag) >> g.rbits) == (uint32_t)(tab[u] >> 32) &&
-                                     r >= r0 && r < r1;
+                                     (CMP || (r >= r0 && r < r1));
                     wi[u] = hit ? r - r0 : 0u;
                     if (HALF) wi[u] += hit && (en[u] & kEntryFlag) ? both0 : 0u;
                     const uint32_t word = rowbits[wi[u] >> 5];
                     need |= (hit && !(word & (1u << (wi[u] & 31)))) ? (1u << u) : 0u;
+                    if constexpr (CMP)
+                        w_hit[wave][__builtin_amdgcn_readfirstlane(e0 - lane) / 64 + u] =
+                            __builtin_amdgcn_ballot_w64(hit && r != q);
                 }
                 if (__any(need != 0)) {
 #pragma unroll
@@ -728,6 +741,18 @@
                 }
             }
             __builtin_amdgcn_wave_barrier();
+            if constexpr (CMP) {
+                for (uint32_t lo = a0 - wb, hi = a1 - wb; a0 < a1 && lo < hi;
+                     lo = (lo | 63u) + 1) {
+                    const uint32_t n = min(hi, (lo | 63u) + 1) - lo;
+                    keptl |= ((w_hit[wave][lo >> 6] >> (lo & 63u)) << (64 - n)) != 0;
+                }
+                __builtin_amdgcn_wave_barrier();
+            }
+        }
+        if constexpr (CMP) {
+            const uint64_t kb = __builtin_amdgcn_ballot_w64(keptl);
+            if (lane == 0) *(uint64_t *)&s_keep[(jb + 256 * bi) >> 5] = kb;
         }
         __builtin_amdgcn_wave_barrier();
       }
@@ -736,6 +761,27 @@
     if (!HALF && events && blockIdx.y == 0 && lane == 0 && ev_w)
         atomicAdd(&events[1 + (blockIdx.x & 63)], ev_w);
     __syncthreads();
+    constexpr int kCp = 4;
+    uint64_t cv[CMP ? kCp : 1];
+    if constexpr (CMP) {
+#pragma unroll
+        for (int u = 0; u < kCp; u++) {
+            const uint32_t i = threadIdx.x + 256 * u;
+            cv[u] = i < lq ? ((const uint64_t *)qry)[rowoff + i] : 0;
+        }
+        if (wave == 3) {
+            const uint32_t c = 2 * lane + 1 < kKeepWords
+                                   ? __popc(s_keep[2 * lane]) + __popc(s_keep[2 * lane + 1]) : 0u;
+            uint32_t inc = c;
+#pragma unroll
+            for (int d = 1; d < 64; d <<= 1) {
+                const uint32_t y = __shfl_up(inc, d, 64);
+                if ((int)lane >= d) inc += y;
+            }
+            s_kpre[lane] = inc - c;
+            if (lane == 63) s_kept = inc;
+        }
+    }
     auto taken = [&](uint32_t w) -> uint32_t {
         const uint32_t m = word_mask(w);
         if (!HALF) return rowbits[w] & m;
@@ -769,6 +815,35 @@
             int t = __builtin_ctz(b);
             b &= b - 1;
             cand[pos++] = bit0 + t;
+        }
+    }
+    if constexpr (CMP) {
+        const uint32_t kept = s_kept;
+        const uint64_t rb = cmp_row_bytes(stride);
+        uint64_t *crow = (uint64_t *)((uint8_t *)cm.rows + (uint64_t)q * rb);
+        uint16_t *cpos = (uint16_t *)((uint8_t *)crow + stride * 8);
+        auto place = [&](uint32_t i, uint64_t v) {
+            uint32_t d = kept + (i - lit);
+            bool keep = true;
+            if (i < lit) {
+                const uint32_t word = s_keep[i >> 5], bit = i & 31;
+                keep = word >> bit & 1u;
+                d = s_kpre[i >> 6] + ((i & 32) ? __popc(s_keep[(i >> 5) - 1]) : 0u) +
+                    __popc(word & ((1u << bit) - 1u));
+            }
+            if (keep) {
+                crow[d] = v;
+                cpos[(d >> 7) * 128 + (d & 63) * 2 + ((d >> 6) & 1)] = (uint16_t)i;
+            }
+        };
+#pragma unroll
+        for (int u = 0; u < kCp; u++)
+            if (threadIdx.x + 256 * u < lq) place(threadIdx.x + 256 * u, cv[u]);
+        for (uint32_t i = threadIdx.x + 256 * kCp; i < lq; i += 256)
+            place(i, ((const uint64_t *)qry)[rowoff + i]);
+        if (threadIdx.x == 0) {
+            cm.len[q] = kept + (lq - lit);
+            cm.len[n_ref + q] = lq;
         }
     }
     if (defaults) {
@@ -949,7 +1024,7 @@
 static hipError_t dyn_lds_attr(int slot, const void *fn, int bytes)
 {
     constexpr int kMaxDev = 64;
-    static std::atomic<int> done[5][kMaxDev];
+    static std::atomic<int> done[7][kMaxDev];
     int dev = 0;
     if (hipError_t e = hipGetDevice(&dev)) return e;
     if (dev < 0 || dev >= kMaxDev) return hipFuncSetAttribute(fn, hipFuncAttributeMaxDynamicSharedMemorySize, bytes);
@@ -1047,9 +1122,12 @@
                              unsigned long long *n_cand, uint64_t *row_seg,
                              const uint32_t *d_qry_it_len, uint32_t *q_unsorted,
                              unsigned long long *events, uint64_t cap, uint32_t *cand_over,
-                             hipStream_t st, uint32_t q_lo, bool half)
+                             hipStream_t st, uint32_t q_lo, bool half, CmpRows cmp)
 {
     if (!n_qry || !n_ref) return hipSuccess;
+    if (cmp.rows && (!half || !cmp.len || hash_bytes != 8 || stride > kCmpMaxRow ||
+                     n_ref > (1u << 19) || q_lo != 0 || n_qry != n_ref))
+        return hipErrorInvalidValue;
     if (half && (!sym || !self_set || g.cut != S || d_qry_it_len || q_unsorted || events))
         return hipErrorInvalidValue;
     const uint32_t chunk = 1u << 19;
@@ -1057,21 +1135,27 @@
     const uint32_t cref = nchunks == 1 ? n_ref : chunk;
     const size_t lds = ((cref + 31) / 32) * 4 * (half ? 2 : 1);
     if (lds > 64 * 1024) {
-        const void *fn = cnt.c16 ? (const void *)probe_rows_kernel<uint16_t, true>
-                                 : (const void *)probe_rows_kernel<uint32_t, true>;
-        if (hipError_t e = dyn_lds_attr(cnt.c16 ? 3 : 4, fn, 128 * 1024)) return e;
+        const void *fn = cmp.rows ? (cnt.c16 ? (const void *)probe_rows_kernel<uint16_t, true, true>
+                                             : (const void *)probe_rows_kernel<uint32_t, true, true>)
+                                  : (cnt.c16 ? (const void *)probe_rows_kernel<uint16_t, true>
+                                             : (const void *)probe_rows_kernel<uint32_t, true>);
+        if (hipError_t e = dyn_lds_attr((cnt.c16 ? 3 : 4) + (cmp.rows ? 2 : 0), fn, 128 * 1024))
+            return e;
     }
     const auto al = [](const void *p) { return ((uintptr_t)p & 15) == 0; };
     const uint32_t vec_defaults = n_ref % 4 == 0 && cref % 4 == 0 && al(d_ref_len) &&
                                   al(cnt.numer) && al(cnt.denom);
-#define FPM_PROBE(C, H)                                                                         \
-    hipLaunchKernelGGL((probe_rows_kernel<C, H>), dim3(xcd_grid(n_qry), nchunks), dim3(256), lds, \
+#define FPM_PROBE(C, ...)                                                                       \
+    hipLaunchKernelGGL((probe_rows_kernel<C, __VA_ARGS__>), dim3(xcd_grid(n_qry), nchunks),      \
+                       dim3(256), lds,                                                           \
                        st, d_qry, d_qry_len, stride, n_qry, q_lo, n_ref, hash_bytes, g, dir,     \
                        entries, cref,                                                            \
                        d_ref_len, S, (uint32_t)sym, (uint32_t)defaults, vec_defaults,           \
                        (uint32_t)self_set, (C *)cnt.numer, (C *)cnt.denom, cand, n_cand, row_seg, \
-                       d_qry_it_len, q_unsorted, events, cap, cand_over)
-    if (cnt.c16 && half) FPM_PROBE(uint16_t, true);
+                       d_qry_it_len, q_unsorted, events, cap, cand_over, cmp)
+    if (cmp.rows && cnt.c16) FPM_PROBE(uint16_t, true, true);
+    else if (cmp.rows) FPM_PROBE(uint32_t, true, true);
+    else if (cnt.c16 && half) FPM_PROBE(uint16_t, true);
     else if (cnt.c16) FPM_PROBE(uint16_t, false);
     else if (half) FPM_PROBE(uint32_t, true);
     else FPM_PROBE(uint32_t, false);
diff --git a/fp-mash_amd/csrc/fpm_ctx.cpp b/fp-mash_amd/csrc/fpm_ctx.cpp
--- a/fp-mash_amd/csrc/fpm_ctx.cpp
+++ b/fp-mash_amd/csrc/fpm_ctx.cpp
@@ -268,6 +268,7 @@
     if (const char *v = getenv("FPM_FILL_COUNTS")) ctx->fill_counts = atoi(v) != 0 ? 1 : 0;
     if (const char *v = getenv("FPM_PROBE_HALF")) ctx->probe_half = atoi(v) != 0;
     if (const char *v = getenv("FPM_INDEX_CUT")) ctx->index_cut = atoi(v) != 0;
+    if (const char *v = getenv("FPM_RANK_COMPACT")) ctx->rank_compact = atoi(v) != 0;
     hipError_t e = hipSetDevice(device);
     if (e == hipSuccess) e = hipStreamCreateWithFlags(&ctx->stream, hipStreamNonBlocking);
     if (e != hipSuccess) {
@@ -498,6 +499,34 @@
     return FPM_OK;
 }
 
+int fpm_ctx_set_rank_compact(fpm_ctx *ctx, int on)
+{
+    if (!ctx) return fail(FPM_EINVAL, "null context");
+    ctx->rank_compact = on != 0;
+    return FPM_OK;
+}
+
+int fpm_ctx_last_rank_compact(fpm_ctx *ctx, int *compact, uint64_t *kept, uint64_t *entries)
+{
+    if (!ctx) return fail(FPM_EINVAL, "null context");
+    if (ctx->last_rank_compact && ctx->last_cmp_len) {
+        if (int rc = set_device(ctx)) return rc;
+        HIP_TRY(hipStreamSynchronize(ctx->last_cmp_stream));
+        std::vector<uint32_t> len(2 * (size_t)ctx->last_cmp_n);
+        HIP_TRY(hipMemcpy(len.data(), ctx->last_cmp_len, len.size() * 4, hipMemcpyDeviceToHost));
+        ctx->last_kept = ctx->last_cmp_entries = 0;
+        for (uint32_t r = 0; r < ctx->last_cmp_n; r++) {
+            ctx->last_kept += len[r];
+            ctx->last_cmp_entries += len[ctx->last_cmp_n + r];
+        }
+        ctx->last_cmp_len = nullptr;
+    }
+    if (compact) *compact = ctx->last_rank_compact ? 1 : 0;
+    if (kept) *kept = ctx->last_rank_compact ? ctx->last_kept : 0;
+    if (entries) *entries = ctx->last_rank_compact ? ctx->last_cmp_entries : 0;
+    return FPM_OK;
+}
+
 int fpm_ctx_index_rebuilds(fpm_ctx *ctx, uint64_t *count)
 {
     if (!ctx || !count) return fail(FPM_EINVAL, "null argument");
diff --git a/fp-mash_amd/csrc/fpm_dist_api.cpp b/fp-mash_amd/csrc/fpm_dist_api.cpp
--- a/fp-mash_amd/csrc/fpm_dist_api.cpp
+++ b/fp-mash_amd/csrc/fpm_dist_api.cpp
@@ -213,6 +213,7 @@
     bool skip_count = false;
     bool spec_probe = false;
     bool spec_half = false;
+    CmpRows spec_cmp{};
     unsigned long long *n_cand() const { return ctr + kCtrCand; }
     uint32_t *unsorted() const { return (uint32_t *)(ctr + kCtrUnsorted); }
     uint32_t *cand_over() const { return (uint32_t *)(ctr + kCtrCandOver); }
@@ -227,6 +228,24 @@
 {
     return c.ctx->index_cut && c.ctx->probe_half && !c.rs && c.self_set && c.hash_bytes == 8 &&
            c.S > 0 && c.R.n <= (1u << 19) && std::max(c.R.stride, c.Q.stride) <= 2048;
+}
+
+static CmpRows compact_rows(const Compare &c, bool half)
+{
+    fpm_ctx *ctx = c.ctx;
+    CmpRows cm;
+    if (!half || !ctx->rank_compact || c.rs || !c.self_set || c.hash_bytes != 8 ||
+        c.R.n > (1u << 19) || c.R.stride > kCmpMaxRow)
+        return cm;
+    void *rows = nullptr, *len = nullptr;
+    if (scratch(ctx, kSlotCmpRows, (size_t)c.R.n * cmp_row_bytes(c.R.stride), &rows) != hipSuccess ||
+        scratch(ctx, kSlotCmpLen, (size_t)c.R.n * 8, &len) != hipSuccess) {
+        (void)hipGetLastError();
+        return cm;
+    }
+    cm.rows = rows;
+    cm.len = (uint32_t *)len;
+    return cm;
 }
 
 static uint64_t whole_index_events(uint64_t ev, uint64_t entries, uint64_t indexed)
@@ -375,11 +394,13 @@
         HIP_TRY(scratch(ctx, kSlotCand, pf.cap * 8, &cand));
         HIP_TRY(scratch(ctx, kSlotRowSeg, (size_t)Q.n * 8, &row_seg));
         p.spec_half = probe_half(c, p, self_set);
+        p.spec_cmp = compact_rows(c, p.spec_half);
         TimedLaunch tl(ctx, FPM_K_PROBE, st);
         HIP_TRY(launch_probe_rows(Q.rows, Q.len, Q.stride, Q.n, R.n, hash_bytes, p.geom, p.dir,
                                   p.entries, R.len, c.S, self_set, pf.defaults, self_set, c.cnt,
                                   (uint64_t *)cand, p.n_cand(), (uint64_t *)row_seg, nullptr,
-                                  nullptr, nullptr, pf.cap, p.cand_over(), st, 0, p.spec_half));
+                                  nullptr, nullptr, pf.cap, p.cand_over(), st, 0, p.spec_half,
+                                  p.spec_cmp));
         tl.done();
         p.spec_probe = true;
         return FPM_OK;
@@ -455,14 +476,18 @@
 }
 
 static hipError_t rank_candidates(const Compare &c, const void *cand, const void *row_seg,
-                                  bool sym, uint32_t *cnum, uint32_t *cden)
+                                  bool sym, uint32_t *cnum, uint32_t *cden, CmpRows cmp = CmpRows{})
 {
     uint32_t rank_cap = 0;
     const hipError_t e =
         launch_merge_rows((const uint64_t *)cand, (const uint64_t *)row_seg, c.Q.n,
                           (const uint64_t *)c.R.rows, c.R.len, c.R.stride, c.R.n,
                           (const uint64_t *)c.Q.rows, c.Q.len, c.Q.stride, c.S, sym, c.cnt, cnum,
-                          cden, c.st, 0, &rank_cap);
+                          cden, c.st, 0, &rank_cap, cmp);
+    c.ctx->last_rank_compact = cmp.rows != nullptr;
+    c.ctx->last_cmp_len = cmp.len;
+    c.ctx->last_cmp_n = c.R.n;
+    c.ctx->last_cmp_stream = c.st;
     c.ctx->last_kernel = rank_cap == 1024 ? FPM_DK_CAND_RANK_1024 : FPM_DK_CAND_RANK_2048;
     return e;
 }
@@ -488,6 +513,7 @@
         ctx->last_events = p.ev;
         cap = std::max<uint64_t>(1, std::min<uint64_t>(p.ev, c.n_pairs));
     }
+    const CmpRows cmp = p.spec_probe ? p.spec_cmp : compact_rows(c, half);
     void *cand, *row_seg;
     HIP_TRY(scratch(ctx, kSlotCand, cap * 8, &cand));
     HIP_TRY(scratch(ctx, kSlotRowSeg, (size_t)Q.n * 8, &row_seg));
@@ -499,7 +525,7 @@
                                   (uint64_t *)row_seg, p.p_len,
                                   p.skip_count ? p.unsorted() : nullptr,
                                   p.skip_count ? p.ctr : nullptr, cap, p.cand_over(), st, 0,
-                                  half));
+                                  half, cmp));
         tl.done();
     }
     bool rank_done = false;
@@ -547,7 +573,7 @@
     if (!rank_done) {
         TimedLaunch tl(ctx, FPM_K_COMPARE, st);
         if (rows_merge)
-            HIP_TRY(rank_candidates(c, cand, row_seg, sym, cnum, cden));
+            HIP_TRY(rank_candidates(c, cand, row_seg, sym, cnum, cden, cmp));
         else {
             HIP_TRY(launch_walk_candidates((const uint64_t *)cand, p.n_cand(), cap, R.rows, R.len,
                                            R.stride, R.n, Q.rows, Q.len, Q.stride, c.hash_bytes,
@@ -643,6 +669,7 @@
     ctx->last_kernel = FPM_DK_NONE;
     ctx->last_probe = FPM_PROBE_NONE;
     ctx->last_index_cut = false;
+    ctx->last_rank_compact = false;
     ctx->last_indexed = ctx->last_entries = 0;
     ctx->last_events = 0;
     ctx->last_cand = 0;
diff --git a/fp-mash_amd/csrc/fpm_internal.hpp b/fp-mash_amd/csrc/fpm_internal.hpp
--- a/fp-mash_amd/csrc/fpm_internal.hpp
+++ b/fp-mash_amd/csrc/fpm_internal.hpp
@@ -120,6 +120,8 @@
     kSlotMergeDescs = 18,
     kSlotRecRefPos = 19,
     kSlotRecQryPos = 20,
+    kSlotCmpRows = 21,
+    kSlotCmpLen = 22,
     kSlotCount
 };
 
@@ -160,6 +162,12 @@
     bool index_cut = true;
     bool last_index_cut = false;
     uint64_t last_indexed = 0, last_entries = 0;
+    bool rank_compact = true;
+    bool last_rank_compact = false;
+    const uint32_t *last_cmp_len = nullptr;
+    uint32_t last_cmp_n = 0;
+    hipStream_t last_cmp_stream = nullptr;
+    uint64_t last_kept = 0, last_cmp_entries = 0;
     int contain_mode = FPM_CONTAIN_AUTO;
     int last_contain_kernel = FPM_CK_NONE;
     int last_screen_kernel = FPM_SK_NONE;
diff --git a/fp-mash_amd/csrc/fpm_kernels.hpp b/fp-mash_amd/csrc/fpm_kernels.hpp
--- a/fp-mash_amd/csrc/fpm_kernels.hpp
+++ b/fp-mash_amd/csrc/fpm_kernels.hpp
@@ -173,6 +173,13 @@
 hipError_t launch_dist_counts_fixup(const uint32_t *d_ref_len, uint32_t n_ref,
                                     const uint32_t *d_qry_len, uint32_t n_qry, uint32_t S,
                                     uint16_t *denom, hipStream_t st);
+struct CmpRows {
+    void *rows = nullptr;
+    uint32_t *len = nullptr;
+};
+constexpr uint64_t cmp_row_bytes(uint64_t stride) { return stride * 8 + (stride + 127) / 128 * 256; }
+constexpr uint32_t kCmpMaxRow = 2048;
+
 hipError_t launch_probe_rows(const void *d_qry, const uint32_t *d_qry_len, uint64_t stride,
                              uint32_t n_qry, uint32_t n_ref, uint32_t hash_bytes, IdxGeom g,
                              const uint32_t *dir, const uint32_t *entries,
@@ -181,13 +188,14 @@
                              unsigned long long *n_cand, uint64_t *row_seg,
                              const uint32_t *d_qry_it_len, uint32_t *q_unsorted,
                              unsigned long long *events, uint64_t cap, uint32_t *cand_over,
-                             hipStream_t st, uint32_t q_lo = 0, bool half = false);
+                             hipStream_t st, uint32_t q_lo = 0, bool half = false,
+                             CmpRows cmp = CmpRows{});
 hipError_t launch_merge_rows(const uint64_t *d_cand, const uint64_t *row_seg, uint32_t n_qry,
                              const uint64_t *d_ref, const uint32_t *d_ref_len, uint64_t ref_stride,
                              uint32_t n_ref, const uint64_t *d_qry, const uint32_t *d_qry_len,
                              uint64_t qry_stride, uint32_t S, bool sym, Counts cnt,
                              uint32_t *d_cnum, uint32_t *d_cden, hipStream_t st, uint32_t q_lo = 0,
-                             uint32_t *rank_cap = nullptr);
+                             uint32_t *rank_cap = nullptr, CmpRows cmp = CmpRows{});
 
 uint32_t text_blocks(uint64_t len);
 uint32_t fp_text_chunk();
diff --git a/fp-mash_amd/fpmash/__init__.py b/fp-mash_amd/fpmash/__init__.py
--- a/fp-mash_amd/fpmash/__init__.py
+++ b/fp-mash_amd/fpmash/__init__.py
@@ -77,6 +77,8 @@
     ("fpm_ctx_last_dist_probe", C.c_int, [vp, C.POINTER(C.c_int)]),
     ("fpm_ctx_set_index_cut", C.c_int, [vp, C.c_int]),
     ("fpm_ctx_last_index_cut", C.c_int, [vp, C.POINTER(C.c_int), u64p, u64p]),
+    ("fpm_ctx_set_rank_compact", C.c_int, [vp, C.c_int]),
+    ("fpm_ctx_last_rank_compact", C.c_int, [vp, C.POINTER(C.c_int), u64p, u64p]),
     ("fpm_sketch_batch", C.c_int, [vp, vp, C.c_char_p, u64p, C.c_uint32, u32p, C.c_uint32,
                                    u64p, u32p]),
     ("fpm_sketch_stage", C.c_int, [vp, vp, C.c_char_p, u64p, C.c_uint32, u32p, C.c_uint32,
@@ -737,6 +739,14 @@
         _check(lib().fpm_ctx_last_index_cut(self.h, C.byref(c), C.byref(i), C.byref(e)))
         return {"cut": bool(c.value), "indexed": i.value, "entries": e.value}
 
+    def set_rank_compact(self, on=True):
+        _check(lib().fpm_ctx_set_rank_compact(self.h, int(on)))
+
+    def last_rank_compact(self):
+        c, k, e = C.c_int(), C.c_uint64(), C.c_uint64()
+        _check(lib().fpm_ctx_last_rank_compact(self.h, C.byref(c), C.byref(k), C.byref(e)))
+        return {"compact": bool(c.value), "kept": k.value, "entries": e.value}
+
     def sketch(self, params, seqs, groups=None, n_groups=None, counts=False, min_copies=1):
         if min_copies != 1:
             r = self.sketch_reads(params, seqs, groups, n_groups, min_copies)
diff --git a/include/fpmash.h b/include/fpmash.h
--- a/include/fpmash.h
+++ b/include/fpmash.h
@@ -91,6 +91,8 @@
 int fpm_ctx_last_dist_probe(fpm_ctx *ctx, int *form);
 int fpm_ctx_set_index_cut(fpm_ctx *ctx, int on);
 int fpm_ctx_last_index_cut(fpm_ctx *ctx, int *cut, uint64_t *indexed, uint64_t *entries);
+int fpm_ctx_set_rank_compact(fpm_ctx *ctx, int on);
+int fpm_ctx_last_rank_compact(fpm_ctx *ctx, int *compact, uint64_t *kept, uint64_t *entries);
 
 int fpm_sketch_batch(fpm_ctx *ctx, const fpm_sketch_params *p, const char *seq,
                      const uint64_t *rec_off, uint32_t n_rec, const uint32_t *group_of_rec,
```

Result: faster. 27.03 billion bases/s, median of 6 (+3.2%).
